# swoonge/SC-A-LOAM

Measured on AMD Instinct MI355X. Metric: scans/sec (feat-extract + scan-to-map ICP + SC loop search), KITTI HDL-64, higher is better.
Workload: dtype f32 points / f64 pose algebra

## Files before the change

sc-a-loam_amd/csrc/common.hpp:

```cpp
#pragma once
#include <hip/hip_runtime.h>
#include <hip/hip_ext.h>
#include <cstdio>
#include <cstdarg>
#include <cstring>
#include <string>
#include <vector>
#include <utility>
#include <mutex>
#include "../../include/scaloam_hip.h"
#include "batch.hpp"

namespace scal {
constexpr unsigned EV_DEVICE_ONLY = hipEventDisableTiming | hipEventDisableSystemFence;


void set_error(const char* fmt, ...);

#define SCAL_HIP(expr)                                                                         \
    do {                                                                                       \
        hipError_t _e = (expr);                                                                \
        if (_e != hipSuccess) {                                                                \
            ::scal::set_error("%s failed: %s (%s:%d)", #expr, hipGetErrorString(_e), __FILE__, __LINE__); \
            return SCAL_E_HIP;                                                                 \
        }                                                                                      \
    } while (0)

#define SCAL_TRY(expr)           \
    do {                         \
        int _rc = (expr);        \
        if (_rc != SCAL_OK) return _rc; \
    } while (0)

int select_device(int device);
enum class StreamLayout { Shared, PerStage };
enum { STAGE_FEATURES = 0, STAGE_SC = 1, STAGE_ODOM = 3, STAGE_MAP = 4, STAGE_MAP_PREFETCH = 2, STAGE_SC_FILTER = 5 };
int stage_lane(StreamLayout layout, int stage);
StreamLayout default_stream_layout();
int acquire_stream(int device, hipStream_t* out, int lane = 0);
void release_stream(int device, int lane = 0);
int odom_create(const scal_odom_config* cfg, StreamLayout layout, scal_odom_t** out);
int map_create(const scal_map_config* cfg, StreamLayout layout, scal_map_t** out);
int sc_create(const scal_sc_config* cfg, StreamLayout layout, scal_sc_t** out);
int icp_create_on_lane(const scal_icp_config* cfg, int lane, scal_icp_t** out);
int refine_create_on_lane(const scal_refine_config* cfg, int lane, scal_refine_t** out);
int posegraph_create_on_lane(const scal_posegraph_config* cfg, int lane, scal_posegraph_t** out);
struct ScFilterOut {
    const float *x, *y, *z, *w;
    const int* d_n;
    int cap;
};
int sc_insert_features_then(scal_sc_t* ctx, scal_features_t* feat, int (*after)(void* user, hipStream_t s, const ScFilterOut& ds), void* user);

struct LaneStream {
    hipStream_t s = nullptr;
    int device = 0, lane = 0;
    LaneStream() = default;
    LaneStream(LaneStream&& o) noexcept { *this = std::move(o); }
    LaneStream& operator=(LaneStream&& o) noexcept {
        release();
        std::swap(s, o.s);
        device = o.device, lane = o.lane;
        return *this;
    }
    ~LaneStream() { release(); }
    operator hipStream_t() const { return s; }
    int acquire(int dev, int ln) {
        release();
        device = dev, lane = ln;
        return acquire_stream(dev, &s, ln);
    }
    void release() {
        if (s) release_stream(device, lane);
        s = nullptr;
    }
};
struct Event {
    hipEvent_t e = nullptr;
    Event() = default;
    Event(Event&& o) noexcept { *this = std::move(o); }
    Event& operator=(Event&& o) noexcept {
        reset();
        std::swap(e, o.e);
        return *this;
    }
    ~Event() { reset(); }
    operator hipEvent_t() const { return e; }
    int create(unsigned flags) {
        reset();
        return ensure(flags);
    }
    int ensure(unsigned flags) {
        const hipError_t r = e ? hipSuccess : hipEventCreateWithFlags(&e, flags);
        if (r == hipSuccess) return SCAL_OK;
        set_error("hipEventCreateWithFlags failed: %s", hipGetErrorString(r));
        e = nullptr;
        return SCAL_E_HIP;
    }
    void reset() {
        if (e) (void)hipEventDestroy(e);
        e = nullptr;
    }
};

template <class T>
struct DevBuf {
    T* p = nullptr;
    size_t n = 0;
    DevBuf() = default;
    DevBuf(const DevBuf&) = delete;
    DevBuf& operator=(const DevBuf&) = delete;
    ~DevBuf() { release(); }
    void release() {
        if (p) (void)hipFree(p);
        p = nullptr;
        n = 0;
    }
    int alloc(size_t count) {
        release();
        if (count == 0) count = 1;
        hipError_t e = hipMalloc(reinterpret_cast<void**>(&p), count * sizeof(T));
        if (e != hipSuccess) {
            set_error("hipMalloc(%zu bytes) failed: %s", count * sizeof(T), hipGetErrorString(e));
            p = nullptr;
            return SCAL_E_HIP;
        }
        n = count;
        return SCAL_OK;
    }
    int zero(hipStream_t s) {
        hipError_t e = op_memset_async(p, 0, n * sizeof(T), s);
        if (e != hipSuccess) {
            set_error("hipMemsetAsync failed: %s", hipGetErrorString(e));
            return SCAL_E_HIP;
        }
        return SCAL_OK;
    }
};

template <class T>
struct PinBuf {
    T* p = nullptr;
    size_t n = 0;
    PinBuf() = default;
    PinBuf(const PinBuf&) = delete;
    PinBuf& operator=(const PinBuf&) = delete;
    ~PinBuf() {
        if (p) (void)hipHostFree(p);
    }
    int alloc(size_t count) {
        if (p) (void)hipHostFree(p);
        p = nullptr;
        if (count == 0) count = 1;
        hipError_t e = hipHostMalloc(reinterpret_cast<void**>(&p), count * sizeof(T), hipHostMallocDefault);
        if (e != hipSuccess) {
            set_error("hipHostMalloc(%zu bytes) failed: %s", count * sizeof(T), hipGetErrorString(e));
            p = nullptr;
            return SCAL_E_HIP;
        }
        n = count;
        return SCAL_OK;
    }
};

inline int div_up(int a, int b) { return (a + b - 1) / b; }

struct HostStage {
    PinBuf<unsigned char> pin;
    size_t used = 0;
    struct Item {
        void* dst;
        size_t off, bytes;
    };
    std::vector<Item> items;
    bool reserve(size_t total) {
        if (pin.p && pin.n >= total) return true;
        if (used) return false;
        if (pin.alloc(total) != SCAL_OK) {
            (void)hipGetLastError();
            return false;
        }
        return true;
    }
    hipError_t d2h(void* user, const void* dev, size_t bytes, hipStream_t s) {
        if (!bytes) return hipSuccess;
        const size_t need = (bytes + 255) & ~static_cast<size_t>(255);
        if (!pin.p || used + need > pin.n) return hipMemcpyAsync(user, dev, bytes, hipMemcpyDeviceToHost, s);
        const hipError_t e = hipMemcpyAsync(pin.p + used, dev, bytes, hipMemcpyDeviceToHost, s);
        items.push_back({user, used, bytes});
        used += need;
        return e;
    }
    hipError_t h2d(void* dev, const void* user, size_t bytes, hipStream_t s) {
        if (!bytes) return hipSuccess;
        const size_t need = (bytes + 255) & ~static_cast<size_t>(255);
        if (!pin.p || used + need > pin.n) return hipMemcpyAsync(dev, user, bytes, hipMemcpyHostToDevice, s);
        std::memcpy(pin.p + used, user, bytes);
        const hipError_t e = hipMemcpyAsync(dev, pin.p + used, bytes, hipMemcpyHostToDevice, s);
        used += need;
        return e;
    }
    void finish() {
        for (const Item& it : items) std::memcpy(it.dst, pin.p + it.off, it.bytes);
        items.clear();
        used = 0;
    }
};

bool prof_begin(const char* name, hipStream_t stream, hipEvent_t* start, hipEvent_t* stop);

#define SCAL_LAUNCH_PROF(name, kernel, grid, block, lds, stream, ...)                                   \
    do {                                                                                                \
        hipEvent_t pe0_ = nullptr, pe1_ = nullptr;                                                      \
        if (::scal::prof_begin(name, stream, &pe0_, &pe1_))                                                     \
            hipExtLaunchKernelGGL(kernel, grid, block, lds, stream, pe0_, pe1_, 0, __VA_ARGS__);        \
        else                                                                                            \
            hipLaunchKernelGGL(kernel, grid, block, lds, stream, __VA_ARGS__);                          \
    } while (0)

}
```

sc-a-loam_amd/csrc/odometry.hip:

```cpp
#include "common.hpp"
#include <deque>
#include "device_utils.hpp"
#include "voxel_dev.hpp"
#include "lm_host.hpp"
#include "features_dev.hpp"
#include <cmath>
#include <algorithm>

namespace scal {

struct OdomCounters {
    int n_corner_last, n_surf_last;
    int n_sharp, n_flat, n_less_sharp, n_less_flat;
    int n_slots, enable;
    int n_live[2], n_edge[2], n_plane[2];
};

__device__ __forceinline__ float sqdist(float ax, float ay, float az, float bx, float by, float bz) {
    return (ax - bx) * (ax - bx) + (ay - by) * (ay - by) + (az - bz) * (az - bz);
}

__device__ __forceinline__ unsigned long long make_key(float d, unsigned seq) {
    return (static_cast<unsigned long long>(__float_as_uint(d)) << 32) | seq;
}

constexpr int RING_TAB = 96;

__device__ __forceinline__ void transform_to_start(const double* x7, float ox, float oy, float oz, float* o) {
    double r[3];
    quat_rotate(x7, static_cast<double>(ox), static_cast<double>(oy), static_cast<double>(oz), r);
    o[0] = static_cast<float>(r[0] + 1.0 * x7[4]);
    o[1] = static_cast<float>(r[1] + 1.0 * x7[5]);
    o[2] = static_cast<float>(r[2] + 1.0 * x7[6]);
}

constexpr int OD_H = 8192;
constexpr int OD_LEVELS = 2;
__device__ constexpr float OD_INV_CELL[OD_LEVELS] = {1.0f, 0.2f};
__device__ constexpr float OD_EXACT_D2[OD_LEVELS] = {0.99f, 24.9f};
struct CellIndex {
    const int* start[OD_LEVELS];
    const float4* pts[OD_LEVELS];
};
__device__ __forceinline__ int od_cell(float v, int level) { return static_cast<int>(floorf(v * OD_INV_CELL[level])); }
__device__ __forceinline__ unsigned od_hash(int cx, int cy, int cz) {
    return (static_cast<unsigned>(cx) * 73856093u ^ static_cast<unsigned>(cy) * 19349663u ^ static_cast<unsigned>(cz) * 83492791u) & (OD_H - 1);
}
__device__ __forceinline__ unsigned od_bucket(float x, float y, float z, int level) { return od_hash(od_cell(x, level), od_cell(y, level), od_cell(z, level)); }
__device__ __forceinline__ unsigned long long od_cell_nn(const int* __restrict__ start, const float4* __restrict__ pts, int level, float sx, float sy, float sz,
                                                          int* s_beg, int* s_pre, unsigned long long* s_nn) {
    const int lane = lane_id(), wv = wave_id();
    if (wv == 0) {
        int b = 0, cnt = 0;
        if (lane < 27) {
            const unsigned h = od_hash(od_cell(sx, level) + lane % 3 - 1, od_cell(sy, level) + (lane / 3) % 3 - 1, od_cell(sz, level) + lane / 9 - 1);
            b = start[h];
            cnt = start[h + 1] - b;
        }
        int incl = cnt;
#pragma unroll
        for (int o = 1; o < 32; o <<= 1) {
            const int v = __shfl_up(incl, o, 64);
            if (lane >= o) incl += v;
        }
        if (lane < 27) s_beg[lane] = b, s_pre[lane + 1] = incl;
        if (lane == 0) s_pre[0] = 0;
    }
    __syncthreads();
    unsigned long long best = ~0ull;
    const int n_cand = s_pre[27];
    for (int m = threadIdx.x; m < n_cand; m += 256) {
        int j = 0;
#pragma unroll
        for (int o = 16; o >= 1; o >>= 1)
            if (j + o <= 26 && s_pre[j + o] <= m) j += o;
        const float4 p = pts[s_beg[j] + (m - s_pre[j])];
        const float dx = sx - p.x, dy = sy - p.y, dz = sz - p.z;
        float d = dx * dx;
        d += dy * dy;
        d += dz * dz;
        best = min(best, make_key(d, __float_as_uint(p.w)));
    }
    best = wave_min_u64(best);
    if (lane == 0) s_nn[wv] = best;
    __syncthreads();
    best = min(min(s_nn[0], s_nn[1]), min(s_nn[2], s_nn[3]));
    __syncthreads();
    return best;
}

__device__ __forceinline__ void k_odom_assoc_body(const CSoA4& sharp, const CSoA4& flat, const CSoA4& CL, const CSoA4& SL, const LMState* __restrict__ st, OdomCounters* C,
                                                    int outer, const FactorSoA& f, const CellIndex& ci_corner, const CellIndex& ci_surf,
                                                    const int* __restrict__ ring_tab) {
    if (!C->enable) return;
    const int ns = C->n_sharp, nf = C->n_flat;
    if (blockIdx.x == 0 && threadIdx.x == 0) C->n_slots = min(ns + nf, f.cap);
    __shared__ unsigned long long s_k2[4], s_k3[4];
    const int q = blockIdx.x;
    if (q >= ns + nf || q >= f.cap) return;
    const int lane = lane_id(), wv = wave_id();
    const bool is_edge = q < ns;
    const int j = is_edge ? q : q - ns;
    const CSoA4& Q = is_edge ? sharp : flat;
    const CSoA4& T = is_edge ? CL : SL;
    const int nT = is_edge ? C->n_corner_last : C->n_surf_last;
    double x7[7];
#pragma unroll
    for (int k = 0; k < 7; ++k) x7[k] = st->x[k];
    const float ox = Q.x[j], oy = Q.y[j], oz = Q.z[j];
    float sel[3];
    transform_to_start(x7, ox, oy, oz, sel);
    const float sx = sel[0], sy = sel[1], sz = sel[2];

    __shared__ int s_beg[27], s_pre[28];
    __shared__ unsigned long long s_nn[4];
    const CellIndex& ci = is_edge ? ci_corner : ci_surf;
    unsigned long long best = od_cell_nn(ci.start[0], ci.pts[0], 0, sx, sy, sz, s_beg, s_pre, s_nn);
    auto dist_of = [](unsigned long long k) { return __uint_as_float(static_cast<unsigned>(k >> 32)); };
    if (best == ~0ull || !(dist_of(best) < OD_EXACT_D2[0])) {
        best = od_cell_nn(ci.start[1], ci.pts[1], 1, sx, sy, sz, s_beg, s_pre, s_nn);
        if (best == ~0ull || !(dist_of(best) < OD_EXACT_D2[1])) {
            best = ~0ull;
            for (int t0 = threadIdx.x; t0 < nT; t0 += 1024) {
                float txx[4], tyy[4], tzz[4];
#pragma unroll
                for (int u = 0; u < 4; ++u) {
                    const int t = min(t0 + 256 * u, nT - 1);
                    txx[u] = T.x[t], tyy[u] = T.y[t], tzz[u] = T.z[t];
                }
#pragma unroll
                for (int u = 0; u < 4; ++u) {
                    const int t = min(t0 + 256 * u, nT - 1);
                    const float dx = sx - txx[u], dy = sy - tyy[u], dz = sz - tzz[u];
                    float d = dx * dx;
                    d += dy * dy;
                    d += dz * dz;
                    best = min(best, make_key(d, static_cast<unsigned>(t)));
                }
            }
            best = wave_min_u64(best);
            if (lane == 0) s_nn[wv] = best;
            __syncthreads();
            best = min(min(s_nn[0], s_nn[1]), min(s_nn[2], s_nn[3]));
        }
    }
    int valid = 0;
    int kind = is_edge ? 0 : 1;
    double pa[3] = {0, 0, 0}, pb[3] = {0, 0, 0};
    const float nnd = __uint_as_float(static_cast<unsigned>(best >> 32));
    if (best != ~0ull && static_cast<double>(nnd) < 25.0) {
        const int c = static_cast<int>(best & 0xffffffffu);
        const int id = static_cast<int>(T.w[c]);
        unsigned long long k2 = ~0ull, k3 = ~0ull;
        const int* first_idx = ring_tab + (is_edge ? 0 : 2 * RING_TAB);
        const int* last_idx = first_idx + RING_TAB;
        int fi = 0x7f7f7f7f, li = -1;
        for (int r = lane; r < RING_TAB; r += 64) {
            if (r >= id + 3) fi = min(fi, first_idx[r]);
            if (r <= id - 3) li = max(li, last_idx[r]);
        }
        const int hi = min(wave_min_i(fi), nT);
        const int lo = wave_max_i(li);
        for (int t0 = c + 1 + lane + 64 * wv; t0 < hi; t0 += 1024) {
            float tw[4], txx[4], tyy[4], tzz[4];
#pragma unroll
            for (int u = 0; u < 4; ++u) {
                const int t = t0 + 256 * u;
                if (t < hi) tw[u] = T.w[t], txx[u] = T.x[t], tyy[u] = T.y[t], tzz[u] = T.z[t];
            }
#pragma unroll
            for (int u = 0; u < 4; ++u) {
                const int t = t0 + 256 * u;
                if (t < hi) {
                    const int rj = static_cast<int>(tw[u]);
                    const float d = sqdist(txx[u], tyy[u], tzz[u], sx, sy, sz);
                    if (static_cast<double>(d) < 25.0) {
                        const unsigned seq = static_cast<unsigned>(t - c - 1);
                        if (is_edge) {
                            if (rj > id) k2 = min(k2, make_key(d, seq));
                        } else {
                            if (rj <= id) k2 = min(k2, make_key(d, seq));
                            else k3 = min(k3, make_key(d, seq));
                        }
                    }
                }
            }
        }
        for (int t0 = c - 1 - lane - 64 * wv; t0 > lo; t0 -= 1024) {
            float tw[4], txx[4], tyy[4], tzz[4];
#pragma unroll
            for (int u = 0; u < 4; ++u) {
                const int t = t0 - 256 * u;
                if (t > lo) tw[u] = T.w[t], txx[u] = T.x[t], tyy[u] = T.y[t], tzz[u] = T.z[t];
            }
#pragma unroll
            for (int u = 0; u < 4; ++u) {
                const int t = t0 - 256 * u;
                if (t > lo) {
                    const int rj = static_cast<int>(tw[u]);
                    const float d = sqdist(txx[u], tyy[u], tzz[u], sx, sy, sz);
                    if (static_cast<double>(d) < 25.0) {
                        const unsigned seq = 0x40000000u + static_cast<unsigned>(c - 1 - t);
                        if (is_edge) {
                            if (rj < id) k2 = min(k2, make_key(d, seq));
                        } else {
                            if (rj >= id) k2 = min(k2, make_key(d, seq));
                            else k3 = min(k3, make_key(d, seq));
                        }
                    }
                }
            }
        }
        k2 = wave_min_u64(k2);
        k3 = wave_min_u64(k3);
        if (lane == 0) s_k2[wv] = k2, s_k3[wv] = k3;
        __syncthreads();
        k2 = min(min(s_k2[0], s_k2[1]), min(s_k2[2], s_k2[3]));
        k3 = min(min(s_k3[0], s_k3[1]), min(s_k3[2], s_k3[3]));
        auto decode = [&](unsigned long long k) {
            const unsigned seq = static_cast<unsigned>(k & 0xffffffffu);
            return (seq & 0x40000000u) ? c - 1 - static_cast<int>(seq & 0x3fffffffu) : c + 1 + static_cast<int>(seq);
        };
        if (is_edge) {
            if (k2 != ~0ull) {
                const int i2 = decode(k2);
                valid = 1;
                pa[0] = T.x[c], pa[1] = T.y[c], pa[2] = T.z[c];
                pb[0] = T.x[i2], pb[1] = T.y[i2], pb[2] = T.z[i2];
            }
        } else if (k2 != ~0ull && k3 != ~0ull) {
            const int i2 = decode(k2), i3 = decode(k3);
            valid = 1;
            const double jx = T.x[c], jy = T.y[c], jz = T.z[c];
            const double lx = T.x[i2], ly = T.y[i2], lz = T.z[i2];
            const double mx = T.x[i3], my = T.y[i3], mz = T.z[i3];
            const double ax = jx - lx, ay = jy - ly, az = jz - lz, bx = jx - mx, by = jy - my, bz = jz - mz;
            double nx = ay * bz - az * by, ny = az * bx - ax * bz, nz = ax * by - ay * bx;
            const double z = nx * nx + ny * ny + nz * nz;
            if (z > 0) {
                const double s = sqrt(z);
                nx /= s, ny /= s, nz /= s;
            }
            pa[0] = jx, pa[1] = jy, pa[2] = jz;
            pb[0] = nx, pb[1] = ny, pb[2] = nz;
        }
    }
    if (lane == 0 && wv == 0) {
        f.valid[q] = valid;
        f.kind[q] = kind;
        f.cp[q] = ox, f.cp[f.cap + q] = oy, f.cp[2 * f.cap + q] = oz;
        f.pa[q] = pa[0], f.pa[f.cap + q] = pa[1], f.pa[2 * f.cap + q] = pa[2];
        f.pb[q] = pb[0], f.pb[f.cap + q] = pb[1], f.pb[2 * f.cap + q] = pb[2];
    }
}
SCAL_KERNEL(256, k_odom_assoc)

__device__ __forceinline__ void k_odom_init_pose_body(LMState* st, int* ring_tab) {
    if (threadIdx.x == 0) {
        st->x[0] = st->x[1] = st->x[2] = 0.0, st->x[3] = 1.0;
        st->x[4] = st->x[5] = st->x[6] = 0.0;
    }
    for (int t = threadIdx.x; t < 8 * RING_TAB; t += blockDim.x) ring_tab[t] = ((t / RING_TAB) & 1) ? -1 : 0x7f7f7f7f;
}
SCAL_KERNEL(1024, k_odom_init_pose)
struct HandoverArgs {
    CSoA4 in[2];
    const int* d_n[2];
    SoA4 out[2];
    int* d_n_out[2];
    int cap[2];
    int nb0;
    int* tab_write;
    int* tab_reset;
    const LMState* st;
    LMState* host_st;
    const LMSync* sync;
    int* cell_cnt[2][OD_LEVELS];
    int* cell_rank[2][OD_LEVELS];
};
__device__ __forceinline__ void k_odom_handover_body(const HandoverArgs& a) {
    int b = blockIdx.x;
    const int k = b < a.nb0 ? 0 : 1;
    if (k) b -= a.nb0;
    if (blockIdx.x == 0) {
        for (int t = threadIdx.x; t < 4 * RING_TAB; t += 256) a.tab_reset[t] = ((t / RING_TAB) & 1) ? -1 : 0x7f7f7f7f;
        const unsigned* src = reinterpret_cast<const unsigned*>(a.st);
        unsigned* dst = reinterpret_cast<unsigned*>(a.host_st);
        const bool abandoned = a.sync->abandoned != 0;
        constexpr int TERM_WORD = static_cast<int>(offsetof(LMState, termination) / 4);
        for (int t = threadIdx.x; t < static_cast<int>(sizeof(LMState) / 4); t += 256) dst[t] = (abandoned && t == TERM_WORD) ? 5u : src[t];
    }
    int* first_idx = a.tab_write + 2 * k * RING_TAB;
    int* last_idx = first_idx + RING_TAB;
    const CSoA4 in = a.in[k];
    const SoA4 out = a.out[k];
    const int n = min(*a.d_n[k], a.cap[k]);
    const int i = b * 256 + threadIdx.x;
    if (i == 0) *a.d_n_out[k] = n;
    if (b * 256 >= n) return;
    const int lane = lane_id();
    float x = 0, y = 0, z = 0;
    if (i < n) {
        const float w = in.w[i];
        x = in.x[i], y = in.y[i], z = in.z[i];
        out.x[i] = x, out.y[i] = y, out.z[i] = z, out.w[i] = w;
        const int r = min(max(static_cast<int>(w), 0), RING_TAB - 1);
        const int rp = __shfl_up(r, 1, 64);
        const int rn = __shfl_down(r, 1, 64);
        if (lane == 0 || rp != r) atomicMin(&first_idx[r], i);
        if (lane == 63 || rn != r || i == n - 1) atomicMax(&last_idx[r], i);
    }
#pragma unroll
    for (int l = 0; l < OD_LEVELS; ++l) {
        const unsigned h = i < n ? od_bucket(x, y, z, l) : 0xffffffffu;
        const unsigned hp = __shfl_up(h, 1, 64);
        const unsigned long long heads = __ballot(lane == 0 || hp != h);
        const int head = 63 - __clzll(heads & (~0ull >> (63 - lane)));
        const unsigned long long above = lane == 63 ? 0ull : heads & (~0ull << (lane + 1));
        const int next = above ? __ffsll(static_cast<long long>(above)) - 1 : 64;
        int base = 0;
        if (lane == head && i < n) {
            base = atomicAdd(&a.cell_cnt[k][l][h], next - head);
        }
        base = __shfl(base, head, 64);
        if (i < n) a.cell_rank[k][l][i] = base + (lane - head);
    }
}
SCAL_KERNEL(256, k_odom_handover)
constexpr int OD_START_STRIDE = OD_H + 4;
__device__ __forceinline__ void k_odom_cellscan_body(int* cnt_all, int* start_all) {
    constexpr int PER = OD_H / 1024;
    static_assert(PER % 4 == 0, "int4 loads");
    int* cnt = cnt_all + blockIdx.x * OD_H;
    int* start = start_all + blockIdx.x * OD_START_STRIDE;
    __shared__ int s_w[16];
    int v[PER];
    int4* c4 = reinterpret_cast<int4*>(cnt + threadIdx.x * PER);
    int sum = 0;
#pragma unroll
    for (int u = 0; u < PER / 4; ++u) {
        const int4 q = c4[u];
        v[4 * u] = q.x, v[4 * u + 1] = q.y, v[4 * u + 2] = q.z, v[4 * u + 3] = q.w;
        sum += q.x + q.y + q.z + q.w;
        c4[u] = make_int4(0, 0, 0, 0);
    }
    int incl = sum;
    const int lane = lane_id(), wv = wave_id();
#pragma unroll
    for (int o = 1; o < 64; o <<= 1) {
        const int t = __shfl_up(incl, o, 64);
        if (lane >= o) incl += t;
    }
    if (lane == 63) s_w[wv] = incl;
    __syncthreads();
    int base = incl - sum;
    for (int w = 0; w < wv; ++w) base += s_w[w];
    int4* s4 = reinterpret_cast<int4*>(start + threadIdx.x * PER);
#pragma unroll
    for (int u = 0; u < PER / 4; ++u) {
        int4 o;
        o.x = base, base += v[4 * u];
        o.y = base, base += v[4 * u + 1];
        o.z = base, base += v[4 * u + 2];
        o.w = base, base += v[4 * u + 3];
        s4[u] = o;
    }
    if (threadIdx.x == 1023) start[OD_H] = base;
}
SCAL_KERNEL(1024, k_odom_cellscan)
struct CellFillArgs {
    CSoA4 in[2];
    const int* d_n[2];
    const int* rank[2][OD_LEVELS];
    const int* start[2][OD_LEVELS];
    float4* pts[2][OD_LEVELS];
    int nb0;
};
__device__ __forceinline__ void k_odom_cellfill_body(const CellFillArgs& a) {
    int b = blockIdx.x;
    const int k = b < a.nb0 ? 0 : 1;
    if (k) b -= a.nb0;
    const int i = b * 256 + threadIdx.x;
    if (i >= *a.d_n[k]) return;
    const float x = a.in[k].x[i], y = a.in[k].y[i], z = a.in[k].z[i];
    const float4 rec = make_float4(x, y, z, __uint_as_float(static_cast<unsigned>(i)));
#pragma unroll
    for (int l = 0; l < OD_LEVELS; ++l) a.pts[k][l][a.start[k][l][od_bucket(x, y, z, l)] + a.rank[k][l][i]] = rec;
}
SCAL_KERNEL(256, k_odom_cellfill)
struct OdomGatherArgs {
    const float *sharp, *flat, *less;
    CSoA4 less_flat;
    const int *n_sharp, *n_flat, *n_less, *n_less_flat;
    SoA4 o_sharp, o_flat, o_less, o_less_flat;
    int slot_cap, feat_cap, cap, nbs, nbf;
};
__device__ __forceinline__ void k_odom_gather_body(const OdomGatherArgs& a, OdomCounters* C) {
    int b = blockIdx.x;
    const float* aos = nullptr;
    const int* d_n;
    int* d_n_out;
    SoA4 out;
    int cap;
    if (b < a.nbs) {
        aos = a.sharp, d_n = a.n_sharp, d_n_out = &C->n_sharp, out = a.o_sharp, cap = a.slot_cap;
        if (b == 0 && threadIdx.x == 0) {
            C->n_slots = 0, C->enable = 1;
            C->n_live[0] = C->n_live[1] = C->n_edge[0] = C->n_edge[1] = C->n_plane[0] = C->n_plane[1] = 0;
        }
    } else if (b < 2 * a.nbs) {
        b -= a.nbs, aos = a.flat, d_n = a.n_flat, d_n_out = &C->n_flat, out = a.o_flat, cap = a.slot_cap;
    } else if (b < 2 * a.nbs + a.nbf) {
        b -= 2 * a.nbs, aos = a.less, d_n = a.n_less, d_n_out = &C->n_less_sharp, out = a.o_less, cap = a.feat_cap;
    } else {
        b -= 2 * a.nbs + a.nbf, d_n = a.n_less_flat, d_n_out = &C->n_less_flat, out = a.o_less_flat, cap = a.cap;
    }
    const int n = min(*d_n, cap);
    const int i = b * 256 + threadIdx.x;
    if (i == 0) *d_n_out = n;
    if (i >= n) return;
    if (aos) {
        const float4 p = reinterpret_cast<const float4*>(aos)[i];
        out.x[i] = p.x, out.y[i] = p.y, out.z[i] = p.z, out.w[i] = p.w;
    } else {
        out.x[i] = a.less_flat.x[i], out.y[i] = a.less_flat.y[i], out.z[i] = a.less_flat.z[i], out.w[i] = a.less_flat.w[i];
    }
}
SCAL_KERNEL(256, k_odom_gather)

}

using namespace scal;

struct scal_odom {
    scal_odom_config cfg;
    LaneStream stream;
    int cap = 0, feat_cap = 0;
    bool systemInited = false;
    static constexpr int MAX_STEPS = 4;
    struct Pending {
        int slot;
        bool solve;
    };
    std::deque<Pending> pending;
    Event ev[MAX_STEPS];
    int next_slot = 0;
    double q_w_curr[4] = {0, 0, 0, 1}, t_w_curr[3] = {0, 0, 0};
    DevBuf<float> aos;
    SoAStore sharp, flat, less_sharp, less_flat;
    SoAStore corner_last, surf_last;
    LMStore lm;
    DevBuf<int> cell_cnt, cell_start, cell_rank;
    DevBuf<float4> cell_pts;
    int* cell_cnt_of(int k, int l) const { return cell_cnt.p + (k * OD_LEVELS + l) * OD_H; }
    int* cell_start_of(int k, int l) const { return cell_start.p + (k * OD_LEVELS + l) * OD_START_STRIDE; }
    int* cell_rank_of(int k, int l) const { return cell_rank.p + (size_t)l * (feat_cap + cap) + (k ? feat_cap : 0); }
    float4* cell_pts_of(int k, int l) const { return cell_pts.p + (size_t)l * (feat_cap + cap) + (k ? feat_cap : 0); }
    CellIndex cell_index(int k) const {
        CellIndex ci;
        for (int l = 0; l < OD_LEVELS; ++l) ci.start[l] = cell_start_of(k, l), ci.pts[l] = cell_pts_of(k, l);
        return ci;
    }
    DevBuf<int> ring_tab;
    int tab_cur = 0;
    DevBuf<OdomCounters> d_C;
    PinBuf<LMState> h_st;
    PinBuf<OdomCounters> h_up;
    HostStage hs;
    bool adapter_active = false, adapter_solve = false;
    BlockAdapter blocks;
    int outer_next = 0;
};

int scal::odom_create(const scal_odom_config* cfg, StreamLayout layout, scal_odom_t** out) {
    if (!cfg || !out || cfg->max_points <= 0) {
        set_error("scal_odom_create: bad argument");
        return SCAL_E_ARG;
    }
    *out = nullptr;
    SCAL_TRY(select_device(cfg->device));
    auto* c = new scal_odom();
    c->cfg = *cfg;
    c->cap = cfg->max_points;
    c->feat_cap = 120 * 64;
    int rc = SCAL_OK;
    auto A = [&](int r) { if (rc == SCAL_OK) rc = r; };
    A(c->lm.alloc(36 * 64));
    A(c->aos.alloc((size_t)c->cap * 4));
    A(c->sharp.alloc(c->lm.slot_cap)); A(c->flat.alloc(c->lm.slot_cap));
    A(c->less_sharp.alloc(c->feat_cap)); A(c->corner_last.alloc(c->feat_cap));
    A(c->less_flat.alloc(c->cap)); A(c->surf_last.alloc(c->cap));
    A(c->cell_cnt.alloc(2 * OD_LEVELS * OD_H)); A(c->cell_start.alloc(2 * OD_LEVELS * OD_START_STRIDE));
    A(c->cell_rank.alloc(OD_LEVELS * ((size_t)c->feat_cap + c->cap))); A(c->cell_pts.alloc(OD_LEVELS * ((size_t)c->feat_cap + c->cap)));
    A(c->ring_tab.alloc(8 * RING_TAB));
    A(c->blocks.alloc(c->lm.slot_cap));
    A(c->d_C.alloc(1)); A(c->h_st.alloc(scal_odom::MAX_STEPS)); A(c->h_up.alloc(1));
    if (rc == SCAL_OK) rc = lm_check_residency<LMNoHook, LMNoHook>(c->cfg.device);
    if (rc == SCAL_OK) rc = c->stream.acquire(c->cfg.device, stage_lane(layout, STAGE_ODOM));
    for (int k = 0; k < scal_odom::MAX_STEPS && rc == SCAL_OK; ++k) rc = c->ev[k].create(hipEventDisableTiming);
    if (rc == SCAL_OK) {
        rc = c->lm.init(c->stream);
        if (rc == SCAL_OK && op_memset_async(c->d_C.p, 0, sizeof(OdomCounters), c->stream) != hipSuccess) rc = SCAL_E_HIP;
        if (rc == SCAL_OK) rc = c->cell_cnt.zero(c->stream);
        if (rc == SCAL_OK) rc = c->cell_start.zero(c->stream);
        SCAL_LAUNCH("k_odom_init_pose", k_odom_init_pose, dim3(1), dim3(256), 0, c->stream, c->lm.d_st.p, c->ring_tab.p);
        if (rc == SCAL_OK && op_stream_synchronize(c->stream) != hipSuccess) rc = SCAL_E_HIP;
    }
    if (rc != SCAL_OK) {
        if (rc == SCAL_E_HIP) set_error("scal_odom_create: HIP resource creation failed");
        delete c;
        return rc;
    }
    *out = c;
    return SCAL_OK;
}

extern "C" int scal_odom_create(const scal_odom_config* cfg, scal_odom_t** out) { return odom_create(cfg, default_stream_layout(), out); }

extern "C" void scal_odom_destroy(scal_odom_t* c) {
    if (!c) return;
    (void)hipSetDevice(c->cfg.device);
    if (c->stream) (void)op_stream_synchronize(c->stream);
    delete c;
}

namespace {

int launch_handover(scal_odom* c, int slot, hipEvent_t ev);
int odom_enqueue(scal_odom* c) {
    hipStream_t s = c->stream;
    OdomCounters* C = c->d_C.p;
    LMState* st = c->lm.d_st.p;
    FactorSoA F = c->lm.factors();
    const bool solve = c->systemInited;
    c->systemInited = true;
    const int slot = c->next_slot;
    c->next_slot = (c->next_slot + 1) % scal_odom::MAX_STEPS;
    if (solve) {
        for (int outer = 0; outer < 2; ++outer) {
            {
                SCAL_LAUNCH("k_odom_assoc", k_odom_assoc, dim3(std::max(1, c->lm.slot_cap)), dim3(256), 0, s, c->sharp.cv(), c->flat.cv(),
                                   c->corner_last.cv(), c->surf_last.cv(), st, C, outer, F, c->cell_index(0), c->cell_index(1), c->ring_tab.p + c->tab_cur * 4 * RING_TAB);
            }
            {
                                launch_lm_solve(s, F, &C->n_slots, st, &C->enable, c->lm.partials.p, c->lm.lm_sync.p, outer, nullptr, LMNoHook(), LMNoHook(), "k_lm_solve_odom");
            }
        }
    }
    SCAL_TRY(launch_handover(c, slot, c->ev[slot]));
    c->pending.push_back({slot, solve});
    return SCAL_OK;
}

int launch_handover(scal_odom* c, int slot, hipEvent_t ev) {
    hipStream_t s = c->stream;
    OdomCounters* C = c->d_C.p;
    LMState* st = c->lm.d_st.p;
    {
        HandoverArgs h;
        h.in[0] = c->less_sharp.cv(), h.in[1] = c->less_flat.cv();
        h.d_n[0] = &C->n_less_sharp, h.d_n[1] = &C->n_less_flat;
        h.out[0] = c->corner_last.v(), h.out[1] = c->surf_last.v();
        h.d_n_out[0] = &C->n_corner_last, h.d_n_out[1] = &C->n_surf_last;
        h.cap[0] = c->feat_cap, h.cap[1] = c->cap;
        h.nb0 = std::max(1, div_up(c->feat_cap, 256));
        h.tab_write = c->ring_tab.p + (c->tab_cur ^ 1) * 4 * RING_TAB;
        h.tab_reset = c->ring_tab.p + c->tab_cur * 4 * RING_TAB;
        h.st = st, h.host_st = c->h_st.p + slot, h.sync = c->lm.lm_sync.p;
        for (int k = 0; k < 2; ++k)
            for (int l = 0; l < OD_LEVELS; ++l) h.cell_cnt[k][l] = c->cell_cnt_of(k, l), h.cell_rank[k][l] = c->cell_rank_of(k, l);
        const dim3 grid(h.nb0 + std::max(1, div_up(c->cap, 256)));
        SCAL_LAUNCH("k_odom_handover", k_odom_handover, grid, dim3(256), 0, s, h);
        c->tab_cur ^= 1;
        if (ev) SCAL_HIP(op_event_record(ev, s));
        SCAL_LAUNCH("k_odom_cellscan", k_odom_cellscan, dim3(2 * OD_LEVELS), dim3(1024), 0, s, c->cell_cnt.p, c->cell_start.p);
        CellFillArgs f;
        f.in[0] = c->corner_last.cv(), f.in[1] = c->surf_last.cv();
        f.d_n[0] = &C->n_corner_last, f.d_n[1] = &C->n_surf_last;
        for (int k = 0; k < 2; ++k)
            for (int l = 0; l < OD_LEVELS; ++l) f.rank[k][l] = c->cell_rank_of(k, l), f.start[k][l] = c->cell_start_of(k, l), f.pts[k][l] = c->cell_pts_of(k, l);
        f.nb0 = h.nb0;
        SCAL_LAUNCH("k_odom_cellfill", k_odom_cellfill, grid, dim3(256), 0, s, f);
    }
    SCAL_HIP(hipGetLastError());
    return SCAL_OK;
}

int odom_collect(scal_odom* c, double* q_lc, double* t_lc, double* q_w, double* t_w, scal_odom_stats* stats) {
    if (c->pending.empty()) {
        set_error("scal_odom_collect: no step enqueued");
        return SCAL_E_STATE;
    }
    const int slot = c->pending.front().slot;
    const bool solve = c->pending.front().solve;
    c->pending.pop_front();
    SCAL_HIP(op_event_synchronize(c->ev[slot]));
    const LMState& L = c->h_st.p[slot];
    if (L.termination == 5) {
        (void)c->lm.clear_exchange(c->stream);
        set_error("LM solve abandoned: grid barrier timed out");
        return SCAL_E_HIP;
    }
    const double* x = L.x;
    if (solve) {
        double r[3];
        q_rot(c->q_w_curr, x + 4, r);
        for (int i = 0; i < 3; ++i) c->t_w_curr[i] = c->t_w_curr[i] + r[i];
        double qn[4];
        q_mul(c->q_w_curr, x, qn);
        for (int i = 0; i < 4; ++i) c->q_w_curr[i] = qn[i];
    }
    for (int i = 0; i < 4; ++i) q_lc[i] = x[i], q_w[i] = c->q_w_curr[i];
    for (int i = 0; i < 3; ++i) t_lc[i] = x[4 + i], t_w[i] = c->t_w_curr[i];
    if (stats) {
        std::memset(stats, 0, sizeof *stats);
        if (solve) {
            for (int o = 0; o < 2; ++o) {
                stats->n_edge[o] = L.log_n_edge[o], stats->n_plane[o] = L.log_n_plane[o];
                stats->lm_iters[o] = L.log_iters[o], stats->lm_success[o] = L.log_success[o];
                stats->cost_init[o] = L.log_cost_init[o], stats->cost_final[o] = L.log_cost_final[o];
            }
        }
    }
    return SCAL_OK;
}

}

static int odom_upload(scal_odom* c, const float* sharp, int n_sharp, const float* less_sharp, int n_less_sharp, const float* flat, int n_flat,
                       const float* less_flat, int n_less_flat) {
    hipStream_t s = c->stream;
    SCAL_HIP(op_stream_synchronize(s));
    c->hs.finish();
    (void)c->hs.reserve(((size_t)2 * c->lm.slot_cap + c->feat_cap + c->cap) * 16 + 4096);
    OdomCounters& H = *c->h_up.p;
    OdomCounters fresh;
    std::memset(&fresh, 0, sizeof fresh);
    fresh.n_sharp = n_sharp, fresh.n_flat = n_flat, fresh.n_less_sharp = n_less_sharp, fresh.n_less_flat = n_less_flat, fresh.enable = 1;
    H = fresh;
    const size_t off = offsetof(OdomCounters, n_sharp);
    SCAL_HIP(op_memcpy_async(reinterpret_cast<char*>(c->d_C.p) + off, reinterpret_cast<char*>(&H) + off, sizeof(OdomCounters) - off,
                            hipMemcpyHostToDevice, s));
    auto up = [&](const float* src, int n, SoAStore& dst) -> int {
        if (n > 0) {
            SCAL_HIP(c->hs.h2d(c->aos.p, src, sizeof(float) * 4 * n, s));
            launch_deinterleave(s, c->aos.p, n, dst.v());
        }
        return SCAL_OK;
    };
    SCAL_TRY(up(sharp, n_sharp, c->sharp));
    SCAL_TRY(up(flat, n_flat, c->flat));
    SCAL_TRY(up(less_sharp, n_less_sharp, c->less_sharp));
    SCAL_TRY(up(less_flat, n_less_flat, c->less_flat));
    return SCAL_OK;
}

extern "C" int scal_odom_step(scal_odom_t* c, const float* sharp, int n_sharp, const float* less_sharp, int n_less_sharp, const float* flat,
                              int n_flat, const float* less_flat, int n_less_flat, double* q_lc, double* t_lc, double* q_w, double* t_w,
                              scal_odom_stats* stats) {
    if (!c || !q_lc || !t_lc || !q_w || !t_w || n_sharp < 0 || n_less_sharp < 0 || n_flat < 0 || n_less_flat < 0 || (n_sharp && !sharp) ||
        (n_less_sharp && !less_sharp) || (n_flat && !flat) || (n_less_flat && !less_flat)) {
        set_error("scal_odom_step: bad argument");
        return SCAL_E_ARG;
    }
    if (n_sharp + n_flat > c->lm.slot_cap || n_sharp > c->lm.slot_cap || n_flat > c->lm.slot_cap || n_less_sharp > c->feat_cap || n_less_flat > c->cap) {
        set_error("scal_odom_step: cloud larger than the context capacity (sharp+flat <= %d, lessSharp <= %d, lessFlat <= %d)", c->lm.slot_cap,
                  c->feat_cap, c->cap);
        return SCAL_E_TOO_MANY;
    }
    SCAL_HIP(hipSetDevice(c->cfg.device));
    if (!c->pending.empty()) {
        set_error("scal_odom_step: a queued step has not been collected");
        return SCAL_E_STATE;
    }
    SCAL_TRY(odom_upload(c, sharp, n_sharp, less_sharp, n_less_sharp, flat, n_flat, less_flat, n_less_flat));
    SCAL_TRY(odom_enqueue(c));
    return odom_collect(c, q_lc, t_lc, q_w, t_w, stats);
}

extern "C" int scal_odom_enqueue_features(scal_odom_t* c, scal_features_t* feat) {
    if (!c || !feat) {
        set_error("scal_odom_enqueue_features: null argument");
        return SCAL_E_ARG;
    }
    if (static_cast<int>(c->pending.size()) >= scal_odom::MAX_STEPS) {
        set_error("scal_odom_enqueue_features: %d steps are queued and not collected", scal_odom::MAX_STEPS);
        return SCAL_E_STATE;
    }
    FeatDeviceView v = features_view(feat);
    if (v.device != c->cfg.device) {
        set_error("features context lives on device %d, odometry context on %d", v.device, c->cfg.device);
        return SCAL_E_ARG;
    }
    SCAL_HIP(hipSetDevice(c->cfg.device));
    hipStream_t s = c->stream;
    OdomGatherArgs a;
    a.sharp = v.sharp_xyzi, a.flat = v.flat_xyzi, a.less = v.less_xyzi;
    a.less_flat = CSoA4{v.lfx, v.lfy, v.lfz, v.lfi};
    a.n_sharp = &v.P->n_sharp, a.n_flat = &v.P->n_flat, a.n_less = &v.P->n_less_sharp, a.n_less_flat = &v.P->n_less_flat;
    a.o_sharp = c->sharp.v(), a.o_flat = c->flat.v(), a.o_less = c->less_sharp.v(), a.o_less_flat = c->less_flat.v();
    a.slot_cap = c->lm.slot_cap, a.feat_cap = c->feat_cap, a.cap = std::min(c->cap, v.cap);
    a.nbs = std::max(1, div_up(c->lm.slot_cap, 256)), a.nbf = std::max(1, div_up(c->feat_cap, 256));
    SCAL_TRY(features_wait_done(feat, s));
    SCAL_LAUNCH("k_odom_gather", k_odom_gather, dim3(2 * a.nbs + a.nbf + std::max(1, div_up(a.cap, 256))), dim3(256), 0, s, a, c->d_C.p);
    SCAL_TRY(features_note_reader(feat, s));
    return odom_enqueue(c);
}

extern "C" int scal_odom_collect(scal_odom_t* c, double* q_lc, double* t_lc, double* q_w, double* t_w, scal_odom_stats* stats) {
    if (!c || !q_lc || !t_lc || !q_w || !t_w) {
        set_error("scal_odom_collect: null argument");
        return SCAL_E_ARG;
    }
    SCAL_HIP(hipSetDevice(c->cfg.device));
    return odom_collect(c, q_lc, t_lc, q_w, t_w, stats);
}

extern "C" int scal_odom_step_features(scal_odom_t* c, scal_features_t* feat, double* q_lc, double* t_lc, double* q_w, double* t_w,
                                       scal_odom_stats* stats) {
    if (!c || !feat || !q_lc || !t_lc || !q_w || !t_w) {
        set_error("scal_odom_step_features: null argument");
        return SCAL_E_ARG;
    }
    SCAL_TRY(scal_odom_enqueue_features(c, feat));
    return odom_collect(c, q_lc, t_lc, q_w, t_w, stats);
}

extern "C" int scal_odom_adapter_begin(scal_odom_t* c, const float* sharp, int n_sharp, const float* less_sharp, int n_less_sharp, const float* flat,
                                       int n_flat, const float* less_flat, int n_less_flat, double* q_last_curr, double* t_last_curr, int* need_solve) {
    if (!c || !q_last_curr || !t_last_curr || !need_solve || n_sharp < 0 || n_less_sharp < 0 || n_flat < 0 || n_less_flat < 0 || (n_sharp && !sharp) ||
        (n_less_sharp && !less_sharp) || (n_flat && !flat) || (n_less_flat && !less_flat)) {
        set_error("scal_odom_adapter_begin: bad argument");
        return SCAL_E_ARG;
    }
    if (n_sharp + n_flat > c->lm.slot_cap || n_less_sharp > c->feat_cap || n_less_flat > c->cap) {
        set_error("scal_odom_adapter_begin: cloud larger than the context capacity");
        return SCAL_E_TOO_MANY;
    }
    if (!c->pending.empty() || c->adapter_active) {
        set_error("scal_odom_adapter_begin: a step is still open");
        return SCAL_E_STATE;
    }
    SCAL_HIP(hipSetDevice(c->cfg.device));
    hipStream_t s = c->stream;
    SCAL_HIP(op_stream_synchronize(s));
    SCAL_TRY(odom_upload(c, sharp, n_sharp, less_sharp, n_less_sharp, flat, n_flat, less_flat, n_less_flat));
    SCAL_HIP(op_memcpy_async(c->h_st.p, c->lm.d_st.p, sizeof(LMState), hipMemcpyDeviceToHost, s));
    SCAL_HIP(op_stream_synchronize(s));
    for (int i = 0; i < 4; ++i) q_last_curr[i] = c->h_st.p->x[i];
    for (int i = 0; i < 3; ++i) t_last_curr[i] = c->h_st.p->x[4 + i];
    c->adapter_solve = c->systemInited;
    c->systemInited = true;
    *need_solve = c->adapter_solve ? 1 : 0;
    c->adapter_active = true;
    c->outer_next = 0;
    return SCAL_OK;
}

extern "C" int scal_odom_associate(scal_odom_t* c, const double* q_last_curr, const double* t_last_curr, int* n_blocks, int* n_residuals) {
    if (!c || !q_last_curr || !t_last_curr || !n_blocks || !n_residuals) {
        set_error("scal_odom_associate: null argument");
        return SCAL_E_ARG;
    }
    if (!c->adapter_active || !c->adapter_solve) {
        set_error("scal_odom_associate: no open step that needs a solve");
        return SCAL_E_STATE;
    }
    SCAL_HIP(hipSetDevice(c->cfg.device));
    hipStream_t s = c->stream;
    OdomCounters* C = c->d_C.p;
    LMState* st = c->lm.d_st.p;
    FactorSoA F = c->lm.factors();
    SCAL_TRY(c->blocks.set_pose(c->stream, c->lm.d_st.p->x, q_last_curr, t_last_curr));
    SCAL_LAUNCH("k_odom_assoc", k_odom_assoc, dim3(std::max(1, c->lm.slot_cap)), dim3(256), 0, s, c->sharp.cv(), c->flat.cv(), c->corner_last.cv(),
                     c->surf_last.cv(), st, C, std::min(c->outer_next, 1), F, c->cell_index(0), c->cell_index(1), c->ring_tab.p + c->tab_cur * 4 * RING_TAB);
    c->outer_next++;
    SCAL_TRY(c->blocks.compact(s, F, &C->n_slots));
    SCAL_HIP(op_stream_synchronize(s));
    *n_blocks = c->blocks.n_blocks(), *n_residuals = c->blocks.n_residuals();
    return SCAL_OK;
}

extern "C" int scal_odom_get_blocks(scal_odom_t* c, scal_block* out, int cap) {
    if (!c || (!out && cap > 0) || cap < 0) {
        set_error("scal_odom_get_blocks: bad argument");
        return SCAL_E_ARG;
    }
    if (!c->adapter_active) {
        set_error("scal_odom_get_blocks: no scal_odom_adapter_begin");
        return SCAL_E_STATE;
    }
    SCAL_HIP(hipSetDevice(c->cfg.device));
    return c->blocks.get_blocks(c->stream, c->lm.factors(), out, cap);
}

extern "C" int scal_odom_eval_blocks(scal_odom_t* c, const double* x7, int want_jac, double* residuals, double* jacobians) {
    if (!c || !x7 || !residuals || (want_jac && !jacobians)) {
        set_error("scal_odom_eval_blocks: bad argument");
        return SCAL_E_ARG;
    }
    if (!c->adapter_active) {
        set_error("scal_odom_eval_blocks: no scal_odom_adapter_begin");
        return SCAL_E_STATE;
    }
    SCAL_HIP(hipSetDevice(c->cfg.device));
    return c->blocks.eval_blocks(c->stream, c->lm.factors(), x7, want_jac, residuals, jacobians);
}

extern "C" int scal_odom_adapter_finish(scal_odom_t* c, const double* q_last_curr, const double* t_last_curr, double* q_w_curr, double* t_w_curr) {
    if (!c || !q_last_curr || !t_last_curr || !q_w_curr || !t_w_curr) {
        set_error("scal_odom_adapter_finish: null argument");
        return SCAL_E_ARG;
    }
    if (!c->adapter_active) {
        set_error("scal_odom_adapter_finish: no scal_odom_adapter_begin");
        return SCAL_E_STATE;
    }
    SCAL_HIP(hipSetDevice(c->cfg.device));
    c->adapter_active = false;
    SCAL_TRY(c->blocks.set_pose(c->stream, c->lm.d_st.p->x, q_last_curr, t_last_curr));
    const int slot = c->next_slot;
    c->next_slot = (c->next_slot + 1) % scal_odom::MAX_STEPS;
    SCAL_TRY(launch_handover(c, slot, c->ev[slot]));
    c->pending.push_back({slot, c->adapter_solve});
    double q_lc[4], t_lc[3];
    return odom_collect(c, q_lc, t_lc, q_w_curr, t_w_curr, nullptr);
}

extern "C" void* scal_odom_stream(scal_odom_t* c) { return c ? static_cast<void*>(c->stream) : nullptr; }
```

sc-a-loam_amd/csrc/pipeline.cpp:

```cpp
#include "common.hpp"
#include "keyframes.hpp"
#include <algorithm>
#include <cmath>
#include <condition_variable>
#include <deque>
#include <chrono>
#include <cstdlib>
#include <string>
#include <thread>

namespace scal {
void print_forced_flushes();
}
using namespace scal;

namespace {
constexpr int REC_N = 64;
constexpr int MAX_UNPOPPED = 32;
constexpr int MAX_LOOPS_UNPOPPED = 64;
int env_int(const char* name, int dflt, int lo, int hi) {
    const char* e = std::getenv(name);
    if (!e) return dflt;
    const int v = std::atoi(e);
    return v < lo ? lo : (v > hi ? hi : v);
}
const int B_AHEAD = env_int("SCALOAM_PIPE_B_AHEAD", 2, 1, 3);
const int PF_AHEAD = env_int("SCALOAM_PIPE_PF_AHEAD", 3, 1, 3);

const bool TIMING = env_int("SCALOAM_PIPE_TIMING", 0, 0, 1) != 0;
struct HostTimer {
    const char* name[12] = {};
    double total[12] = {};
    long calls[12] = {};
    template <class F>
    int run(int slot, const char* nm, F&& f) {
        if (!TIMING) return f();
        const auto t0 = std::chrono::steady_clock::now();
        const int rc = f();
        name[slot] = nm;
        total[slot] += std::chrono::duration<double, std::micro>(std::chrono::steady_clock::now() - t0).count();
        calls[slot]++;
        return rc;
    }
    void print(const char* thread) const {
        for (int i = 0; i < 12; ++i)
            if (calls[i]) std::fprintf(stderr, "[scal_pipeline] %-6s %-28s %8.1f us/call x %ld\n", thread, name[i], total[i] / calls[i], calls[i]);
    }
};

constexpr int SMAX = scal::BATCH_MAX;
struct Rec {
    const float* d_xyz[SMAX] = {};
    const void* h_xyz[SMAX] = {};
    int n[SMAX] = {};
    int stride = 0;
    bool host = false;
    scal_pipeline_result res[SMAX] = {};
};
}

struct scal_pipeline {
    scal_pipeline_config cfg{};
    int ring = 6, depth = 2;
    int S = 1;
    std::vector<scal_features_t*> regs[SMAX];
    scal_odom_t* od[SMAX] = {};
    scal_map_t* mp[SMAX] = {};
    scal_sc_t* sc[SMAX] = {};
    double* d_desc = nullptr;
    bool own_desc = false;
    Rec rec[REC_N];
    std::mutex mu;
    std::condition_variable cv;
    long long pushed = 0, a_run = 0, a_done = 0, pf_done = 0, b_enq = 0, b_coll = 0, c_enq = 0, c_coll = 0, d_ins = 0, d_coll = 0, popped = 0;
    int pop_waiting = 0;
    bool drain_req = false, drained = true;
    bool stop = false;
    int err = SCAL_OK;
    std::string errmsg;
    std::thread t_front, t_side, t_odom, t_pose, t_loop;
    HostTimer tm_front, tm_side, tm_odom, tm_pose, tm_loop;
    KeyframeStore* kf = nullptr;
    scal_keyframe_gate_state gate{};
    double fitness_thres = 0.3;
    std::deque<KfLoopJob> jobs;
    std::deque<scal_pipeline_loop> loops;
    bool verifying = false;
    long long verifying_seq = 0;
    long long loops_owed = 0;
    std::thread t_verify;
    struct AcceptedLoop {
        int curr_kf, loop_kf;
        double q[4], t[3];
    };
    std::vector<AcceptedLoop> accepted;
    int verifying_kf = -1;
    int kf_passed_end = 0;
    scal_posegraph_t* pg = nullptr;

    bool sc_on() const { return cfg.sc_mode != SCAL_PIPE_SC_OFF; }
    bool side_sc() const { return cfg.sc_mode == SCAL_PIPE_SC_EVERY_SCAN || cfg.sc_mode == SCAL_PIPE_SC_DESCRIPTOR; }
    bool kf_mode() const { return cfg.sc_mode == SCAL_PIPE_SC_KEYFRAME; }
    bool verify_idle() const { return jobs.empty() && !verifying; }
    Rec& r(long long k) { return rec[k % REC_N]; }
    template <class F>
    int for_all(F&& f) {
        if (S == 1) return f(0);
        Recorder recs[SMAX];
        Recorder* ptr[SMAX];
        int rc = SCAL_OK;
        for (int q = 0; q < S && rc == SCAL_OK; ++q) {
            ptr[q] = &recs[q];
            g_recorder = &recs[q];
            rc = f(q);
            g_recorder = nullptr;
        }
        if (rc != SCAL_OK) {
            for (int q = 0; q < S; ++q) (void)recs[q].flush();
            return rc;
        }
        if (zip_and_launch(ptr, S) != hipSuccess) {
            set_error("scal_pipeline: a batched launch failed: %s", hipGetErrorString(hipGetLastError()));
            return SCAL_E_HIP;
        }
        return SCAL_OK;
    }
    template <class F>
    int for_each(F&& f) {
        for (int q = 0; q < S; ++q) SCAL_TRY(f(q));
        return SCAL_OK;
    }
    void fail(int rc) {
        if (err == SCAL_OK) {
            err = rc;
            errmsg = scal_last_error();
        }
        cv.notify_all();
    }
};

namespace {

void front_thread(scal_pipeline* p) {
    std::unique_lock<std::mutex> lk(p->mu);
    for (;;) {
        const long long k = p->a_done;
        p->cv.wait(lk, [&] {
            if (p->stop || p->err) return true;
            if (p->pushed <= k) return false;
            const long long old = k - p->ring;
            if (old >= 0 && (p->c_coll <= old || p->b_enq <= old || (p->sc_on() && p->d_ins <= old))) return false;
            return k - p->c_enq < PF_AHEAD;
        });
        if (p->stop || p->err) return;
        const Rec& rc = p->r(k);
        const int slot = static_cast<int>(k % p->ring);
        lk.unlock();
        int st = p->tm_front.run(0, "A: features_run", [&] {
            return p->for_all([&](int q) {
                scal_features_t* reg = p->regs[q][slot];
                return rc.host ? scal_features_enqueue_host(reg, rc.h_xyz[q], rc.n[q], rc.stride) : scal_features_run_device(reg, rc.d_xyz[q], rc.n[q], rc.stride);
            });
        });
        if (st == SCAL_OK) {
            lk.lock();
            p->a_run = k + 1;
            p->cv.notify_all();
            lk.unlock();
            st = p->tm_front.run(1, "C: prefetch, lane 0 half", [&] { return p->for_all([&](int q) { return scal_map_prefetch_begin(p->mp[q], p->regs[q][slot]); }); });
        }
        lk.lock();
        if (st != SCAL_OK) {
            p->fail(st);
            return;
        }
        p->a_done = k + 1;
        p->cv.notify_all();
    }
}

void side_thread(scal_pipeline* p) {
    std::unique_lock<std::mutex> lk(p->mu);
    const bool search = p->cfg.sc_mode == SCAL_PIPE_SC_EVERY_SCAN;
    for (;;) {
        const long long k = p->pf_done;
        p->cv.wait(lk, [&] {
            if (p->stop || p->err) return true;
            if (p->a_done <= k) return false;
            return !(p->side_sc() && k - p->d_coll >= 3);
        });
        if (p->stop || p->err) return;
        const int slot = static_cast<int>(k % p->ring);
        lk.unlock();
        double* dd = p->d_desc ? p->d_desc + static_cast<size_t>(slot) * 1200 : nullptr;
        int st = p->tm_side.run(1, "C: prefetch, side half + D: insert", [&]() -> int {
            if (!p->side_sc() && p->S == 1) return scal_map_prefetch_finish(p->mp[0], p->regs[0][slot]);
            Recorder recs[2 * SMAX];
            Recorder* ptr[2 * SMAX];
            int nr = 0, rc2 = SCAL_OK;
            rc2 = p->tm_side.run(3, "   record prefetch", [&] {
                int r3 = SCAL_OK;
                for (int q = 0; q < p->S && r3 == SCAL_OK; ++q) {
                    g_recorder = ptr[nr] = &recs[nr];
                    ++nr;
                    r3 = scal_map_prefetch_finish(p->mp[q], p->regs[q][slot]);
                    g_recorder = nullptr;
                }
                return r3;
            });
            if (rc2 == SCAL_OK && p->side_sc())
                rc2 = p->tm_side.run(4, "   record insert", [&] {
                    int r3 = SCAL_OK;
                    for (int q = 0; q < p->S && r3 == SCAL_OK; ++q) {
                        g_recorder = ptr[nr] = &recs[nr];
                        ++nr;
                        r3 = search ? scal_sc_insert_features(p->sc[q], p->regs[q][slot]) : scal_sc_make_features_enqueue(p->sc[q], p->regs[q][slot], dd);
                        g_recorder = nullptr;
                    }
                    return r3;
                });
            if (rc2 != SCAL_OK) {
                for (int i = 0; i < nr; ++i) (void)recs[i].flush();
                return rc2;
            }
            return p->tm_side.run(5, "   zip + launch", [&]() -> int {
                if (zip_marked_and_launch(ptr, nr) != hipSuccess) {
                    set_error("scal_pipeline: a batched launch failed: %s", hipGetErrorString(hipGetLastError()));
                    return SCAL_E_HIP;
                }
                return SCAL_OK;
            });
        });
        if (st == SCAL_OK && search) st = p->tm_side.run(2, "D: sc_detect_enqueue", [&] { return p->for_all([&](int q) { return scal_sc_detect_enqueue(p->sc[q]); }); });
        lk.lock();
        if (st != SCAL_OK) {
            p->fail(st);
            return;
        }
        p->r(k).res[0].d_descriptor = dd;
        p->pf_done = k + 1;
        if (p->side_sc()) p->d_ins = k + 1;
        p->cv.notify_all();
    }
}

void odom_thread(scal_pipeline* p) {
    std::unique_lock<std::mutex> lk(p->mu);
    for (;;) {
        enum { NONE, B_ENQ, B_COLL } what = NONE;
        p->cv.wait(lk, [&] {
            if (p->stop || p->err) return true;
            if (p->b_enq < p->a_run && p->b_enq - p->b_coll < B_AHEAD) { what = B_ENQ; return true; }
            if (p->b_coll < p->b_enq && p->b_coll - p->c_enq < 2) { what = B_COLL; return true; }
            return false;
        });
        if (p->stop || p->err) return;
        int st = SCAL_OK;
        if (what == B_ENQ) {
            const long long k = p->b_enq;
            const int slot = static_cast<int>(k % p->ring);
            lk.unlock();
            st = p->tm_odom.run(0, "B: odom_enqueue_features", [&] { return p->for_all([&](int q) { return scal_odom_enqueue_features(p->od[q], p->regs[q][slot]); }); });
            lk.lock();
            if (st == SCAL_OK) p->b_enq = k + 1;
        } else {
            const long long k = p->b_coll;
            scal_pipeline_result* R = p->r(k).res;
            lk.unlock();
            st = p->tm_odom.run(1, "B: odom_collect (wait)", [&] {
                return p->for_each([&](int q) {
                    double qlc[4], tlc[3];
                    return scal_odom_collect(p->od[q], qlc, tlc, R[q].q_odom, R[q].t_odom, &R[q].odom);
                });
            });
            lk.lock();
            if (st == SCAL_OK) p->b_coll = k + 1;
        }
        if (st != SCAL_OK) {
            p->fail(st);
            return;
        }
        p->cv.notify_all();
    }
}

void pose_thread(scal_pipeline* p) {
    std::unique_lock<std::mutex> lk(p->mu);
    for (;;) {
        enum { NONE, C_ENQ, C_COLL, FINISH } what = NONE;
        p->cv.wait(lk, [&] {
            if (p->stop || p->err) return true;
            const long long inflight = p->c_enq - p->c_coll;
            if (p->c_enq < p->b_coll && p->c_enq < p->pf_done && inflight <= p->depth) { what = C_ENQ; return true; }
            if (inflight > p->depth || (inflight > 0 && (p->pop_waiting || p->drain_req) && p->c_enq == p->pushed)) { what = C_COLL; return true; }
            if (p->drain_req && p->c_coll == p->pushed) { what = FINISH; return true; }
            return false;
        });
        if (p->stop || p->err) return;
        int st = SCAL_OK;
        if (what == C_ENQ) {
            const long long k = p->c_enq;
            const int slot = static_cast<int>(k % p->ring);
            scal_pipeline_result* R = p->r(k).res;
            lk.unlock();
            st = p->tm_pose.run(2, "C: map_enqueue_features", [&] {
                return p->for_all([&](int q) { return scal_map_enqueue_features(p->mp[q], p->regs[q][slot], R[q].q_odom, R[q].t_odom); });
            });
            lk.lock();
            if (st == SCAL_OK) p->c_enq = k + 1;
        } else if (what == C_COLL) {
            const long long k = p->c_coll;
            scal_pipeline_result* R = p->r(k).res;
            lk.unlock();
            st = p->tm_pose.run(3, "C: map_collect (wait)", [&] {
                return p->for_each([&](int q) { return scal_map_collect(p->mp[q], R[q].q_w_curr, R[q].t_w_curr, &R[q].map); });
            });
            lk.lock();
            if (st == SCAL_OK) p->c_coll = k + 1;
        } else if (what == FINISH) {
            lk.unlock();
            st = p->for_each([&](int q) { return scal_map_finish(p->mp[q]); });
            lk.lock();
            if (st == SCAL_OK) p->drain_req = false, p->drained = true;
        }
        if (st != SCAL_OK) {
            p->fail(st);
            return;
        }
        p->cv.notify_all();
    }
}

void loop_thread(scal_pipeline* p) {
    std::unique_lock<std::mutex> lk(p->mu);
    const bool search = p->cfg.sc_mode == SCAL_PIPE_SC_EVERY_SCAN;
    for (;;) {
        p->cv.wait(lk, [&] {
            if (p->stop || p->err) return true;
            const long long infl = p->d_ins - p->d_coll;
            return infl >= 2 || (infl > 0 && (p->pop_waiting || p->drain_req));
        });
        if (p->stop || p->err) return;
        const long long k = p->d_coll;
        scal_pipeline_result* R = p->r(k).res;
        lk.unlock();
        int st;
        if (search) {
            st = p->tm_loop.run(2, "D: sc_detect_collect (wait)", [&] {
                return p->for_each([&](int q) {
                    const int rc = scal_sc_detect_collect(p->sc[q], &R[q].loop);
                    R[q].have_loop = rc == SCAL_OK;
                    return rc;
                });
            });
        } else {
            st = scal_sc_wait_descriptor(p->sc[0]);
        }
        lk.lock();
        if (st != SCAL_OK) {
            p->fail(st);
            return;
        }
        p->d_coll = k + 1;
        p->cv.notify_all();
    }
}

void keyframe_thread(scal_pipeline* p) {
    std::unique_lock<std::mutex> lk(p->mu);
    for (;;) {
        const long long k = p->d_coll;
        p->cv.wait(lk, [&] { return p->stop || p->err || p->c_coll > k; });
        if (p->stop || p->err) return;
        scal_pipeline_result& R = p->r(k).res[0];
        const int slot = static_cast<int>(k % p->ring);
        lk.unlock();
        int is_kf = 0;
        bool detect = false;
        int st = scal_keyframe_gate(&p->gate, R.q_w_curr, R.t_w_curr, &is_kf);
        R.is_keyframe = is_kf, R.keyframe_id = -1, R.have_loop = 0;
        if (st == SCAL_OK && is_kf) {
            const int id = scal_sc_size(p->sc[0]);
            double p6[6];
            pose6_from(R.q_w_curr, R.t_w_curr, p6);
            st = p->tm_loop.run(0, "D: insert + append", [&] { return p->kf->insert(p->sc[0], p->regs[0][slot], id, p6); });
            if (st == SCAL_OK) {
                R.keyframe_id = id;
                detect = p->kf->own_count() >= 30;
                if (detect) st = p->tm_loop.run(1, "D: sc_detect_enqueue", [&] { return scal_sc_detect_enqueue(p->sc[0]); });
            }
        }
        lk.lock();
        if (st != SCAL_OK) {
            p->fail(st);
            return;
        }
        p->d_ins = k + 1;
        p->cv.notify_all();
        lk.unlock();
        if (detect) {
            st = p->tm_loop.run(2, "D: sc_detect_collect (wait)", [&] { return scal_sc_detect_collect(p->sc[0], &R.loop); });
            R.have_loop = st == SCAL_OK;
        }
        if (st == SCAL_OK && is_kf) st = p->kf->check();
        lk.lock();
        if (st != SCAL_OK) {
            p->fail(st);
            return;
        }
        if (detect && R.loop.loop_id >= 0) {
            p->jobs.push_back(KfLoopJob{k, R.keyframe_id, R.loop.loop_id, R.loop.yaw_rad, R.loop.min_dist});
            p->loops_owed++;
        }
        if (is_kf) p->kf_passed_end = R.keyframe_id + 1;
        p->d_coll = k + 1;
        p->cv.notify_all();
    }
}

void verify_thread(scal_pipeline* p) {
    std::unique_lock<std::mutex> lk(p->mu);
    for (;;) {
        p->cv.wait(lk, [&] { return p->stop || p->err || !p->jobs.empty(); });
        if (p->stop || p->err) return;
        const KfLoopJob job = p->jobs.front();
        p->jobs.pop_front();
        p->verifying = true, p->verifying_seq = job.seq, p->verifying_kf = job.curr_kf;
        lk.unlock();
        scal_pipeline_loop rec;
        const int st = p->kf->verify(job, p->fitness_thres, &rec);
        lk.lock();
        p->verifying = false;
        if (st != SCAL_OK) {
            p->fail(st);
            return;
        }
        p->loops.push_back(rec);
        if (rec.verified == 1) {
            scal_pipeline::AcceptedLoop a{rec.curr_kf, rec.loop_kf, {rec.q_rel[0], rec.q_rel[1], rec.q_rel[2], rec.q_rel[3]}, {rec.t_rel[0], rec.t_rel[1], rec.t_rel[2]}};
            p->accepted.push_back(a);
        }
        p->cv.notify_all();
    }
}

int report(scal_pipeline* p) {
    set_error("%s", p->errmsg.c_str());
    return p->err;
}

int push(scal_pipeline* p, const float* const* d_xyz, const void* const* h_xyz, const int* n, int stride, bool host) {
    std::unique_lock<std::mutex> lk(p->mu);
    if (p->err) return report(p);
    if (p->pushed - p->popped >= MAX_UNPOPPED) {
        set_error("scal_pipeline_push: %d results wait to be popped", MAX_UNPOPPED);
        return SCAL_E_STATE;
    }
    if (p->loops_owed >= MAX_LOOPS_UNPOPPED) {
        set_error("scal_pipeline_push: %d loop records wait to be popped (scal_pipeline_pop_loop)", MAX_LOOPS_UNPOPPED);
        return SCAL_E_STATE;
    }
    const long long k = p->pushed;
    Rec& rc = p->r(k);
    rc = Rec();
    for (int q = 0; q < p->S; ++q) {
        rc.d_xyz[q] = d_xyz ? d_xyz[q] : nullptr, rc.h_xyz[q] = h_xyz ? h_xyz[q] : nullptr, rc.n[q] = n[q];
        rc.res[q].seq = k;
    }
    rc.stride = stride, rc.host = host;
    p->pushed = k + 1;
    p->drained = false;
    p->cv.notify_all();
    p->cv.wait(lk, [&] { return p->err || (host ? p->a_done > k : p->a_done + p->ring > k); });
    if (p->err) return report(p);
    return SCAL_OK;
}

int pop(scal_pipeline* p, scal_pipeline_result* out) {
    std::unique_lock<std::mutex> lk(p->mu);
    if (p->popped >= p->pushed && !p->err) {
        set_error("scal_pipeline_pop: nothing pushed");
        return SCAL_E_STATE;
    }
    const long long k = p->popped;
    p->pop_waiting++;
    p->cv.notify_all();
    p->cv.wait(lk, [&] { return p->err || (p->c_coll > k && (!p->sc_on() || p->d_coll > k)); });
    p->pop_waiting--;
    if (p->err) return report(p);
    for (int q = 0; q < p->S; ++q) out[q] = p->r(k).res[q];
    p->popped = k + 1;
    p->cv.notify_all();
    return SCAL_OK;
}

int create(const scal_pipeline_config* cfg, int n_seqs, scal_pipeline_t** out) {
    if (!cfg || !out) {
        set_error("scal_pipeline_create: null argument");
        return SCAL_E_ARG;
    }
    *out = nullptr;
    const int ring = cfg->ring == 0 ? 6 : cfg->ring, depth = cfg->depth == 0 ? 2 : cfg->depth;
    if (ring < 4 || ring > 16 || depth < 1 || depth > 3 || cfg->sc_mode < 0 || cfg->sc_mode > 3) {
        set_error("scal_pipeline_create: ring must be 4..16, depth 1..3, sc_mode 0..3");
        return SCAL_E_ARG;
    }
    if (n_seqs < 1 || n_seqs > SMAX || (n_seqs > 1 && (cfg->sc_mode == SCAL_PIPE_SC_DESCRIPTOR || cfg->sc_mode == SCAL_PIPE_SC_KEYFRAME))) {
        set_error("scal_pipeline_create_multi: 1..%d sequences (sc_mode 2 and 3 only with one)", SMAX);
        return SCAL_E_ARG;
    }
    scal_keyframe_gate_state gate{};
    if (cfg->sc_mode == SCAL_PIPE_SC_KEYFRAME) {
        if (cfg->kf_max_points < 0 || !(cfg->loop_fitness_thres >= 0) || cfg->sc_max_keyframes <= 0 ||
            scal_keyframe_gate_init(&gate, cfg->keyframe_meter_gap == 0 ? 2.0 : cfg->keyframe_meter_gap,
                                    cfg->keyframe_deg_gap == 0 ? 10.0 : cfg->keyframe_deg_gap) != SCAL_OK) {
            set_error("scal_pipeline_create: sc_mode 3 needs keyframe gaps >= 0, kf_max_points >= 0, loop_fitness_thres >= 0, sc_max_keyframes > 0");
            return SCAL_E_ARG;
        }
    }
    if (cfg->pgo_map_max_points < 0 || (cfg->pgo_map_max_points > 0 && (cfg->sc_mode != SCAL_PIPE_SC_KEYFRAME || cfg->kf_max_points == 0))) {
        set_error("scal_pipeline_create: pgo_map_max_points must be >= 0, and > 0 only in sc_mode 3 with kf_max_points > 0");
        return SCAL_E_ARG;
    }
    SCAL_TRY(select_device(cfg->device));
    auto* p = new scal_pipeline();
    p->cfg = *cfg, p->ring = ring, p->depth = depth, p->S = n_seqs;
    p->gate = gate;
    p->fitness_thres = cfg->loop_fitness_thres == 0 ? 0.3 : cfg->loop_fitness_thres;
    int rc = SCAL_OK;
    if (p->kf_mode()) {
        p->kf = new KeyframeStore();
        rc = p->kf->init(cfg->device, cfg->kf_max_points, cfg->sc_max_keyframes, cfg->pgo_map_max_points);
    }
    scal_features_config fc{};
    fc.lidar_type = cfg->lidar_type, fc.n_scans = cfg->n_scans, fc.minimum_range = cfg->minimum_range, fc.max_points = cfg->max_points;
    fc.float_math = cfg->float_math, fc.check_finite = cfg->check_finite, fc.device = cfg->device;
    for (int q = 0; q < n_seqs && rc == SCAL_OK; ++q) {
        for (int i = 0; i < ring && rc == SCAL_OK; ++i) {
            scal_features_t* f = nullptr;
            rc = scal_features_create(&fc, &f);
            if (rc == SCAL_OK) p->regs[q].push_back(f);
        }
        if (rc == SCAL_OK) {
            scal_odom_config oc{};
            oc.max_points = cfg->max_points, oc.device = cfg->device;
            rc = odom_create(&oc, StreamLayout::PerStage, &p->od[q]);
        }
        if (rc == SCAL_OK) {
            scal_map_config mc{};
            mc.line_res = cfg->line_res, mc.plane_res = cfg->plane_res, mc.max_scan_points = cfg->max_points, mc.max_map_points = cfg->max_map_points;
            mc.device = cfg->device;
            rc = map_create(&mc, StreamLayout::PerStage, &p->mp[q]);
        }
        if (rc == SCAL_OK && p->sc_on()) {
            scal_sc_config sc{};
            sc.max_radius = cfg->sc_max_radius, sc.dist_thres = cfg->sc_dist_thres, sc.max_keyframes = cfg->sc_max_keyframes;
            sc.float_math = cfg->float_math, sc.device = cfg->device, sc.n_shards = 1, sc.shard = 0, sc.side_stream = env_int("SCALOAM_PIPE_SC_LANE", 1, 0, 5);
            rc = sc_create(&sc, StreamLayout::PerStage, &p->sc[q]);
            if (rc == SCAL_OK && cfg->sc_mode == SCAL_PIPE_SC_DESCRIPTOR) {
                if (cfg->d_desc_ring) {
                    p->d_desc = cfg->d_desc_ring;
                } else if (hipMalloc(reinterpret_cast<void**>(&p->d_desc), sizeof(double) * 1200 * ring) != hipSuccess) {
                    set_error("scal_pipeline_create: hipMalloc of the descriptor ring failed");
                    rc = SCAL_E_HIP;
                } else {
                    p->own_desc = true;
                }
            }
        }
    }
    if (rc != SCAL_OK) {
        const std::string keep = scal_last_error();
        scal_pipeline_destroy(p);
        set_error("%s", keep.c_str());
        return rc;
    }
    p->t_front = std::thread(front_thread, p);
    p->t_side = std::thread(side_thread, p);
    p->t_odom = std::thread(odom_thread, p);
    p->t_pose = std::thread(pose_thread, p);
    if (p->side_sc()) p->t_loop = std::thread(loop_thread, p);
    if (p->kf_mode()) p->t_loop = std::thread(keyframe_thread, p), p->t_verify = std::thread(verify_thread, p);
    *out = p;
    return SCAL_OK;
}

}

extern "C" int scal_pipeline_create(const scal_pipeline_config* cfg, scal_pipeline_t** out) { return create(cfg, 1, out); }
extern "C" int scal_pipeline_create_multi(const scal_pipeline_config* cfg, int n_seqs, scal_pipeline_t** out) { return create(cfg, n_seqs, out); }
extern "C" int scal_pipeline_seqs(scal_pipeline_t* p) { return p ? p->S : 0; }

extern "C" void scal_pipeline_destroy(scal_pipeline_t* p) {
    if (!p) return;
    {
        std::lock_guard<std::mutex> lk(p->mu);
        p->stop = true;
        p->cv.notify_all();
    }
    if (p->t_front.joinable()) p->t_front.join();
    if (p->t_side.joinable()) p->t_side.join();
    if (p->t_odom.joinable()) p->t_odom.join();
    if (p->t_pose.joinable()) p->t_pose.join();
    if (p->t_loop.joinable()) p->t_loop.join();
    if (p->t_verify.joinable()) p->t_verify.join();
    if (TIMING) {
        p->tm_front.print("front"), p->tm_side.print("side"), p->tm_odom.print("odom"), p->tm_pose.print("pose"), p->tm_loop.print("loop");
        std::fprintf(stderr, "[scal_pipeline] sequences %d, recorded lists flushed in the middle of an entry point: %ld\n", p->S, g_forced_flushes);
        print_forced_flushes();
    }
    (void)hipSetDevice(p->cfg.device);
    for (int q = 0; q < SMAX; ++q) {
        if (p->sc[q]) scal_sc_destroy(p->sc[q]);
        if (p->mp[q]) scal_map_destroy(p->mp[q]);
        if (p->od[q]) scal_odom_destroy(p->od[q]);
    }
    for (int q = 0; q < SMAX; ++q)
        for (auto* f : p->regs[q]) scal_features_destroy(f);
    if (p->pg) scal_posegraph_destroy(p->pg);
    delete p->kf;
    if (p->d_desc && p->own_desc) (void)hipFree(p->d_desc);
    delete p;
}

static int check_scan(scal_pipeline_t* p, const void* ptr, int n) {
    if ((!ptr && n > 0) || n < 0) {
        set_error("scal_pipeline_push: bad argument");
        return SCAL_E_ARG;
    }
    if (n > p->cfg.max_points) {
        set_error("scan has %d points, capacity is %d", n, p->cfg.max_points);
        return SCAL_E_TOO_MANY;
    }
    return SCAL_OK;
}

extern "C" int scal_pipeline_push_device(scal_pipeline_t* p, const float* d_xyz, int n, int stride_floats) {
    if (!p || stride_floats < 3 || p->S != 1) {
        set_error("scal_pipeline_push_device: bad argument (a pipeline of several sequences takes scal_pipeline_push_device_multi)");
        return SCAL_E_ARG;
    }
    SCAL_TRY(check_scan(p, d_xyz, n));
    return push(p, &d_xyz, nullptr, &n, stride_floats, false);
}

extern "C" int scal_pipeline_push_device_multi(scal_pipeline_t* p, const float* const* d_xyz, const int* n, int stride_floats) {
    if (!p || !d_xyz || !n || stride_floats < 3) {
        set_error("scal_pipeline_push_device_multi: bad argument");
        return SCAL_E_ARG;
    }
    for (int q = 0; q < p->S; ++q) SCAL_TRY(check_scan(p, d_xyz[q], n[q]));
    return push(p, d_xyz, nullptr, n, stride_floats, false);
}

extern "C" int scal_pipeline_push_host(scal_pipeline_t* p, const void* xyz, int n, int stride_bytes) {
    if (!p || stride_bytes < 12 || (stride_bytes % 4) != 0 || stride_bytes > 32 || p->S != 1) {
        set_error("scal_pipeline_push_host: bad argument (stride_bytes must be a multiple of 4 in [12, 32]; one sequence)");
        return SCAL_E_ARG;
    }
    SCAL_TRY(check_scan(p, xyz, n));
    return push(p, nullptr, &xyz, &n, stride_bytes, true);
}

extern "C" int scal_pipeline_pop(scal_pipeline_t* p, scal_pipeline_result* out) {
    if (!p || !out || p->S != 1) {
        set_error("scal_pipeline_pop: bad argument (a pipeline of several sequences takes scal_pipeline_pop_multi)");
        return SCAL_E_ARG;
    }
    return pop(p, out);
}

extern "C" int scal_pipeline_pop_multi(scal_pipeline_t* p, scal_pipeline_result* out) {
    if (!p || !out) {
        set_error("scal_pipeline_pop_multi: null argument");
        return SCAL_E_ARG;
    }
    return pop(p, out);
}

extern "C" int scal_pipeline_drain(scal_pipeline_t* p) {
    if (!p) return SCAL_E_ARG;
    std::unique_lock<std::mutex> lk(p->mu);
    if (p->err) return report(p);
    if (p->drained) return SCAL_OK;
    p->drain_req = true;
    p->pop_waiting++;
    p->cv.notify_all();
    p->cv.wait(lk, [&] { return p->err || (p->drained && (!p->sc_on() || p->d_coll == p->pushed) && p->verify_idle()); });
    p->pop_waiting--;
    if (p->err) return report(p);
    return SCAL_OK;
}

extern "C" int scal_pipeline_pop_loop(scal_pipeline_t* p, scal_pipeline_loop* out, int wait) {
    if (!p || !out) {
        set_error("scal_pipeline_pop_loop: null argument");
        return SCAL_E_ARG;
    }
    std::unique_lock<std::mutex> lk(p->mu);
    if (!p->kf_mode()) {
        set_error("scal_pipeline_pop_loop: only in sc_mode 3");
        return SCAL_E_STATE;
    }
    for (;;) {
        if (p->err) return report(p);
        if (!p->loops.empty()) {
            *out = p->loops.front();
            p->loops.pop_front();
            p->loops_owed--;
            return 1;
        }
        if (!wait || p->verify_idle()) return 0;
        p->cv.wait(lk);
    }
}

extern "C" int scal_pipeline_keyframe(scal_pipeline_t* p, int kf, double pose6[6], float* xyzi, int cap, int* n) {
    if (!p || !pose6 || !n || cap < 0 || (cap > 0 && !xyzi)) {
        set_error("scal_pipeline_keyframe: bad argument");
        return SCAL_E_ARG;
    }
    std::lock_guard<std::mutex> lk(p->mu);
    if (p->err) return report(p);
    if (!p->kf_mode() || !p->drained || p->d_coll != p->pushed || !p->verify_idle()) {
        set_error("scal_pipeline_keyframe: only in sc_mode 3, while the pipeline is drained");
        return SCAL_E_STATE;
    }
    return p->kf->read(kf, pose6, xyzi, cap, n);
}

static int update_poses_locked(scal_pipeline_t* p, const int* kf, const double* pose6, int n);

extern "C" int scal_pipeline_update_keyframe_poses(scal_pipeline_t* p, const int* kf, const double* pose6, int n) {
    if (!p || n < 0 || (n > 0 && (!kf || !pose6))) {
        set_error("scal_pipeline_update_keyframe_poses: bad argument");
        return SCAL_E_ARG;
    }
    std::lock_guard<std::mutex> lk(p->mu);
    if (p->err) return report(p);
    if (!p->kf_mode()) {
        set_error("scal_pipeline_update_keyframe_poses: only in sc_mode 3");
        return SCAL_E_STATE;
    }
    return update_poses_locked(p, kf, pose6, n);
}

static int update_poses_locked(scal_pipeline_t* p, const int* kf, const double* pose6, int n) {
    long long floor = p->d_coll;
    if (!p->jobs.empty()) floor = std::min(floor, p->jobs.front().seq);
    if (p->verifying) floor = std::min(floor, p->verifying_seq);
    return p->kf->update_poses(kf, pose6, n, p->pushed, floor);
}

static int pgo_map_state(scal_pipeline_t* p) {
    std::lock_guard<std::mutex> lk(p->mu);
    if (p->err) return report(p);
    if (!p->kf_mode() || p->cfg.pgo_map_max_points == 0) {
        set_error("scal_pipeline_pgo_map: only in sc_mode 3 with pgo_map_max_points > 0");
        return SCAL_E_STATE;
    }
    return SCAL_OK;
}

extern "C" int scal_pipeline_pgo_map(scal_pipeline_t* p, int kf_end, int skip, float leaf, float* out_xyzi, long long cap, long long* n_out) {
    if (!p || !n_out || cap < 0 || (cap > 0 && !out_xyzi)) {
        set_error("scal_pipeline_pgo_map: bad argument");
        return SCAL_E_ARG;
    }
    *n_out = 0;
    SCAL_TRY(pgo_map_state(p));
    if (!(leaf > 0.f) || !std::isfinite(leaf) || skip < 1 || kf_end < 0) {
        set_error("scal_pipeline_pgo_map: leaf must be finite and > 0, skip >= 1, kf_end >= 0");
        return SCAL_E_ARG;
    }
    return p->kf->pgo_map(kf_end, skip, leaf, out_xyzi, cap, n_out);
}

extern "C" const float* scal_pipeline_pgo_map_device(scal_pipeline_t* p, long long* n) {
    if (n) *n = 0;
    if (!p || !n || !p->kf_mode() || p->cfg.pgo_map_max_points == 0) return nullptr;
    return p->kf->pgo_map_device(n);
}

namespace {
void pose7_from6(const double* p6, double* p7) {
    const double cr = std::cos(p6[3] / 2), sr = std::sin(p6[3] / 2), cp = std::cos(p6[4] / 2), sp = std::sin(p6[4] / 2);
    const double cy = std::cos(p6[5] / 2), sy = std::sin(p6[5] / 2);
    p7[0] = sr * cp * cy - cr * sp * sy, p7[1] = cr * sp * cy + sr * cp * sy, p7[2] = cr * cp * sy - sr * sp * cy, p7[3] = cr * cp * cy + sr * sp * sy;
    p7[4] = p6[0], p7[5] = p6[1], p7[6] = p6[2];
}
void pose7_between(const double* a, const double* b, double* o) {
    const double x = -a[0], y = -a[1], z = -a[2], w = a[3];
    o[0] = w * b[0] + x * b[3] + y * b[2] - z * b[1];
    o[1] = w * b[1] - x * b[2] + y * b[3] + z * b[0];
    o[2] = w * b[2] + x * b[1] - y * b[0] + z * b[3];
    o[3] = w * b[3] - x * b[0] - y * b[1] - z * b[2];
    const double d[3] = {b[4] - a[4], b[5] - a[5], b[6] - a[6]};
    const double R[3][3] = {{1 - 2 * (y * y + z * z), 2 * (x * y - w * z), 2 * (x * z + w * y)},
                            {2 * (x * y + w * z), 1 - 2 * (x * x + z * z), 2 * (y * z - w * x)},
                            {2 * (x * z - w * y), 2 * (y * z + w * x), 1 - 2 * (x * x + y * y)}};
    for (int r = 0; r < 3; ++r) o[4 + r] = (R[r][0] * d[0] + R[r][1] * d[1]) + R[r][2] * d[2];
}
}

extern "C" int scal_pipeline_optimize_keyframes(scal_pipeline_t* p, int kf_end, int apply, int* kf_ids, double* pose6, int cap, scal_pipeline_pgo_result* res) {
    if (res) std::memset(res, 0, sizeof *res);
    if (!p || cap < 0 || (cap > 0 && (!kf_ids || !pose6))) {
        set_error("scal_pipeline_optimize_keyframes: bad argument");
        return SCAL_E_ARG;
    }
    {
        std::lock_guard<std::mutex> lk(p->mu);
        if (p->err) return report(p);
        if (!p->kf_mode()) {
            set_error("scal_pipeline_optimize_keyframes: only in sc_mode 3");
            return SCAL_E_STATE;
        }
    }
    if (kf_end < 0) {
        set_error("scal_pipeline_optimize_keyframes: kf_end must be >= 0");
        return SCAL_E_ARG;
    }
    std::vector<int> ids;
    std::vector<std::array<double, 6>> gated, current;
    SCAL_TRY(p->kf->pgo_snapshot(kf_end, &ids, &gated, &current));
    const int n = static_cast<int>(ids.size());
    if (res) res->n_nodes = n;
    if (cap < n) {
        set_error("scal_pipeline_optimize_keyframes: %d keyframes, room for %d", n, cap);
        return SCAL_E_CAPACITY;
    }
    if (n == 0) return SCAL_OK;
    std::vector<scal_pipeline::AcceptedLoop> loops;
    {
        std::unique_lock<std::mutex> lk(p->mu);
        const int need = ids.back() + 1;
        auto pending = [&] {
            if (p->verifying && p->verifying_kf < kf_end) return true;
            for (const KfLoopJob& j : p->jobs)
                if (j.curr_kf < kf_end) return true;
            return false;
        };
        p->cv.wait(lk, [&] { return p->err || p->stop || (p->kf_passed_end >= need && !pending()); });
        if (p->err) return report(p);
        if (p->stop) {
            set_error("scal_pipeline_optimize_keyframes: the pipeline is being destroyed");
            return SCAL_E_STATE;
        }
        for (const auto& a : p->accepted)
            if (a.curr_kf < kf_end) loops.push_back(a);
    }
    std::vector<double> x7(7 * static_cast<size_t>(n)), g7(7 * static_cast<size_t>(n));
    scal_posegraph_stats st{};
    {
        std::lock_guard<std::mutex> map_lk(p->kf->map_mu);
        SCAL_TRY(p->kf->pgo_snapshot(kf_end, &ids, &gated, &current));
        for (int k = 0; k < n; ++k) pose7_from6(gated[static_cast<size_t>(k)].data(), &g7[7 * static_cast<size_t>(k)]), pose7_from6(current[static_cast<size_t>(k)].data(), &x7[7 * static_cast<size_t>(k)]);
        if (!p->pg) {
            scal_posegraph_config pc{};
            pc.device = p->cfg.device, pc.max_nodes = p->cfg.sc_max_keyframes, pc.max_edges = 2 * p->cfg.sc_max_keyframes;
            SCAL_TRY(posegraph_create_on_lane(&pc, 2, &p->pg));
        }
        const double var_prior[6] = {1e-12, 1e-12, 1e-12, 1e-12, 1e-12, 1e-12};
        const double var_odom[6] = {1e-6, 1e-6, 1e-6, 1e-4, 1e-4, 1e-4};
        const double var_loop[6] = {0.5, 0.5, 0.5, 0.5, 0.5, 0.5};
        const size_t m = static_cast<size_t>(n - 1) + loops.size();
        std::vector<int> ei(m), ej(m);
        std::vector<double> ez(7 * m), ev(6 * m), ek(m);
        for (int k = 1; k < n; ++k) {
            const size_t e = static_cast<size_t>(k - 1);
            ei[e] = k - 1, ej[e] = k, ek[e] = 0.0;
            pose7_between(&g7[7 * e], &g7[7 * (e + 1)], &ez[7 * e]);
            std::memcpy(&ev[6 * e], var_odom, sizeof var_odom);
        }
        size_t e = static_cast<size_t>(n - 1);
        for (const auto& a : loops) {
            const auto node = [&](int db) { return static_cast<int>(std::lower_bound(ids.begin(), ids.end(), db) - ids.begin()); };
            ei[e] = node(a.loop_kf), ej[e] = node(a.curr_kf), ek[e] = 1.0;
            std::memcpy(&ez[7 * e], a.q, sizeof a.q), std::memcpy(&ez[7 * e + 4], a.t, sizeof a.t);
            std::memcpy(&ev[6 * e], var_loop, sizeof var_loop);
            ++e;
        }
        SCAL_TRY(scal_posegraph_set_nodes(p->pg, x7.data(), n));
        SCAL_TRY(scal_posegraph_clear_edges(p->pg));
        SCAL_TRY(scal_posegraph_set_prior(p->pg, 0, g7.data(), var_prior));
        SCAL_TRY(scal_posegraph_add_between(p->pg, static_cast<int>(m), ei.data(), ej.data(), ez.data(), ev.data(), ek.data()));
        SCAL_TRY(scal_posegraph_optimize(p->pg, nullptr, &st));
        SCAL_TRY(scal_posegraph_get_nodes(p->pg, x7.data(), n));
    }
    for (int k = 0; k < n; ++k) {
        kf_ids[k] = ids[static_cast<size_t>(k)];
        pose6_from(&x7[7 * static_cast<size_t>(k)], &x7[7 * static_cast<size_t>(k) + 4], pose6 + 6 * static_cast<size_t>(k));
    }
    if (res) res->n_odom_edges = n - 1, res->n_loop_edges = static_cast<int>(loops.size()), res->solver = st;
    if (apply) {
        std::lock_guard<std::mutex> lk(p->mu);
        if (p->err) return report(p);
        SCAL_TRY(update_poses_locked(p, kf_ids, pose6, n));
        if (res) res->applied = 1;
    }
    return SCAL_OK;
}

extern "C" int scal_pipeline_in_flight(scal_pipeline_t* p) {
    if (!p) return 0;
    std::lock_guard<std::mutex> lk(p->mu);
    return static_cast<int>(p->pushed - p->popped);
}

static bool seq_ok(scal_pipeline_t* p, int q) { return p && q >= 0 && q < p->S; }
extern "C" scal_sc_t* scal_pipeline_sc(scal_pipeline_t* p) { return p ? p->sc[0] : nullptr; }
extern "C" scal_map_t* scal_pipeline_map(scal_pipeline_t* p) { return p ? p->mp[0] : nullptr; }
extern "C" scal_odom_t* scal_pipeline_odom(scal_pipeline_t* p) { return p ? p->od[0] : nullptr; }
extern "C" scal_features_t* scal_pipeline_features(scal_pipeline_t* p, int i) {
    return (p && i >= 0 && i < static_cast<int>(p->regs[0].size())) ? p->regs[0][i] : nullptr;
}
extern "C" scal_sc_t* scal_pipeline_sc_of(scal_pipeline_t* p, int seq) { return seq_ok(p, seq) ? p->sc[seq] : nullptr; }
extern "C" scal_map_t* scal_pipeline_map_of(scal_pipeline_t* p, int seq) { return seq_ok(p, seq) ? p->mp[seq] : nullptr; }
```

Baseline: 4360.

## Prepare odometry target sets in front thread with ring of sets and paired batched launches

```diff
diff --git a/sc-a-loam_amd/csrc/common.hpp b/sc-a-loam_amd/csrc/common.hpp
--- a/sc-a-loam_amd/csrc/common.hpp
+++ b/sc-a-loam_amd/csrc/common.hpp
@@ -42,6 +42,9 @@
 int odom_create(const scal_odom_config* cfg, StreamLayout layout, scal_odom_t** out);
 int map_create(const scal_map_config* cfg, StreamLayout layout, scal_map_t** out);
 int sc_create(const scal_sc_config* cfg, StreamLayout layout, scal_sc_t** out);
+constexpr int ODOM_TARGET_SETS = 4;
+int odom_prepare_features(scal_odom_t* ctx, scal_features_t* feat, bool own_stream, long long scan);
+int odom_enqueue_prepared(scal_odom_t* ctx);
 int icp_create_on_lane(const scal_icp_config* cfg, int lane, scal_icp_t** out);
 int refine_create_on_lane(const scal_refine_config* cfg, int lane, scal_refine_t** out);
 int posegraph_create_on_lane(const scal_posegraph_config* cfg, int lane, scal_posegraph_t** out);
diff --git a/sc-a-loam_amd/csrc/odometry.hip b/sc-a-loam_amd/csrc/odometry.hip
--- a/sc-a-loam_amd/csrc/odometry.hip
+++ b/sc-a-loam_amd/csrc/odometry.hip
@@ -1,4 +1,5 @@
 #include "common.hpp"
+#include <atomic>
 #include <deque>
 #include "device_utils.hpp"
 #include "voxel_dev.hpp"
@@ -10,10 +11,10 @@
 namespace scal {
 
 struct OdomCounters {
-    int n_corner_last, n_surf_last;
+    int n_slots, enable;
+};
+struct SetCounts {
     int n_sharp, n_flat, n_less_sharp, n_less_flat;
-    int n_slots, enable;
-    int n_live[2], n_edge[2], n_plane[2];
 };
 
 __device__ __forceinline__ float sqdist(float ax, float ay, float az, float bx, float by, float bz) {
@@ -90,10 +91,10 @@
 }
 
 __device__ __forceinline__ void k_odom_assoc_body(const CSoA4& sharp, const CSoA4& flat, const CSoA4& CL, const CSoA4& SL, const LMState* __restrict__ st, OdomCounters* C,
-                                                    int outer, const FactorSoA& f, const CellIndex& ci_corner, const CellIndex& ci_surf,
+                                                    const SetCounts* __restrict__ nq, const SetCounts* __restrict__ nt, int outer, const FactorSoA& f, const CellIndex& ci_corner, const CellIndex& ci_surf,
                                                     const int* __restrict__ ring_tab) {
     if (!C->enable) return;
-    const int ns = C->n_sharp, nf = C->n_flat;
+    const int ns = nq->n_sharp, nf = nq->n_flat;
     if (blockIdx.x == 0 && threadIdx.x == 0) C->n_slots = min(ns + nf, f.cap);
     __shared__ unsigned long long s_k2[4], s_k3[4];
     const int q = blockIdx.x;
@@ -103,7 +104,7 @@
     const int j = is_edge ? q : q - ns;
     const CSoA4& Q = is_edge ? sharp : flat;
     const CSoA4& T = is_edge ? CL : SL;
-    const int nT = is_edge ? C->n_corner_last : C->n_surf_last;
+    const int nT = is_edge ? nt->n_less_sharp : nt->n_less_flat;
     double x7[7];
 #pragma unroll
     for (int k = 0; k < 7; ++k) x7[k] = st->x[k];
@@ -255,55 +256,64 @@
 }
 SCAL_KERNEL(256, k_odom_assoc)
 
-__device__ __forceinline__ void k_odom_init_pose_body(LMState* st, int* ring_tab) {
+constexpr int OD_SETS = ODOM_TARGET_SETS;
+__device__ __forceinline__ void k_odom_init_pose_body(LMState* st, int* ring_tab, OdomCounters* C) {
     if (threadIdx.x == 0) {
         st->x[0] = st->x[1] = st->x[2] = 0.0, st->x[3] = 1.0;
         st->x[4] = st->x[5] = st->x[6] = 0.0;
-    }
-    for (int t = threadIdx.x; t < 8 * RING_TAB; t += blockDim.x) ring_tab[t] = ((t / RING_TAB) & 1) ? -1 : 0x7f7f7f7f;
+        C->n_slots = 0, C->enable = 1;
+    }
+    for (int t = threadIdx.x; t < OD_SETS * 4 * RING_TAB; t += blockDim.x) ring_tab[t] = ((t / RING_TAB) & 1) ? -1 : 0x7f7f7f7f;
 }
 SCAL_KERNEL(1024, k_odom_init_pose)
-struct HandoverArgs {
-    CSoA4 in[2];
-    const int* d_n[2];
-    SoA4 out[2];
-    int* d_n_out[2];
-    int cap[2];
-    int nb0;
-    int* tab_write;
-    int* tab_reset;
-    const LMState* st;
-    LMState* host_st;
-    const LMSync* sync;
+struct OdomPrepArgs {
+    const float *sharp, *flat, *less;
+    const float* less_flat_aos;
+    CSoA4 less_flat;
+    const int *n_sharp, *n_flat, *n_less, *n_less_flat;
+    int n_host[4];
+    SoA4 o_sharp, o_flat, o_less, o_less_flat;
+    SetCounts* cnt;
+    int slot_cap, feat_cap, cap, nbs, nbf;
+    int* tab;
     int* cell_cnt[2][OD_LEVELS];
     int* cell_rank[2][OD_LEVELS];
 };
-__device__ __forceinline__ void k_odom_handover_body(const HandoverArgs& a) {
+__device__ __forceinline__ void k_odom_prepare_body(const OdomPrepArgs& a) {
     int b = blockIdx.x;
-    const int k = b < a.nb0 ? 0 : 1;
-    if (k) b -= a.nb0;
-    if (blockIdx.x == 0) {
-        for (int t = threadIdx.x; t < 4 * RING_TAB; t += 256) a.tab_reset[t] = ((t / RING_TAB) & 1) ? -1 : 0x7f7f7f7f;
-        const unsigned* src = reinterpret_cast<const unsigned*>(a.st);
-        unsigned* dst = reinterpret_cast<unsigned*>(a.host_st);
-        const bool abandoned = a.sync->abandoned != 0;
-        constexpr int TERM_WORD = static_cast<int>(offsetof(LMState, termination) / 4);
-        for (int t = threadIdx.x; t < static_cast<int>(sizeof(LMState) / 4); t += 256) dst[t] = (abandoned && t == TERM_WORD) ? 5u : src[t];
-    }
-    int* first_idx = a.tab_write + 2 * k * RING_TAB;
+    const float* aos = nullptr;
+    const int* d_n;
+    int n_host, cap, k = -1;
+    int* d_n_out;
+    SoA4 out;
+    if (b < a.nbs) {
+        aos = a.sharp, d_n = a.n_sharp, n_host = a.n_host[0], d_n_out = &a.cnt->n_sharp, out = a.o_sharp, cap = a.slot_cap;
+    } else if (b < 2 * a.nbs) {
+        b -= a.nbs, aos = a.flat, d_n = a.n_flat, n_host = a.n_host[1], d_n_out = &a.cnt->n_flat, out = a.o_flat, cap = a.slot_cap;
+    } else if (b < 2 * a.nbs + a.nbf) {
+        b -= 2 * a.nbs, aos = a.less, d_n = a.n_less, n_host = a.n_host[2], d_n_out = &a.cnt->n_less_sharp, out = a.o_less, cap = a.feat_cap, k = 0;
+    } else {
+        b -= 2 * a.nbs + a.nbf, aos = a.less_flat_aos, d_n = a.n_less_flat, n_host = a.n_host[3], d_n_out = &a.cnt->n_less_flat, out = a.o_less_flat, cap = a.cap, k = 1;
+    }
+    const int n = min(d_n ? *d_n : n_host, cap);
+    const int i = b * 256 + threadIdx.x;
+    if (i == 0) *d_n_out = n;
+    if (b * 256 >= n) return;
+    float x = 0, y = 0, z = 0, w = 0;
+    if (i < n) {
+        if (aos) {
+            const float4 p = reinterpret_cast<const float4*>(aos)[i];
+            x = p.x, y = p.y, z = p.z, w = p.w;
+        } else {
+            x = a.less_flat.x[i], y = a.less_flat.y[i], z = a.less_flat.z[i], w = a.less_flat.w[i];
+        }
+        out.x[i] = x, out.y[i] = y, out.z[i] = z, out.w[i] = w;
+    }
+    if (k < 0) return;
+    int* first_idx = a.tab + 2 * k * RING_TAB;
     int* last_idx = first_idx + RING_TAB;
-    const CSoA4 in = a.in[k];
-    const SoA4 out = a.out[k];
-    const int n = min(*a.d_n[k], a.cap[k]);
-    const int i = b * 256 + threadIdx.x;
-    if (i == 0) *a.d_n_out[k] = n;
-    if (b * 256 >= n) return;
     const int lane = lane_id();
-    float x = 0, y = 0, z = 0;
     if (i < n) {
-        const float w = in.w[i];
-        x = in.x[i], y = in.y[i], z = in.z[i];
-        out.x[i] = x, out.y[i] = y, out.z[i] = z, out.w[i] = w;
         const int r = min(max(static_cast<int>(w), 0), RING_TAB - 1);
         const int rp = __shfl_up(r, 1, 64);
         const int rn = __shfl_down(r, 1, 64);
@@ -326,7 +336,17 @@
         if (i < n) a.cell_rank[k][l][i] = base + (lane - head);
     }
 }
-SCAL_KERNEL(256, k_odom_handover)
+SCAL_KERNEL(256, k_odom_prepare)
+__device__ __forceinline__ void k_odom_publish_body(int* tab_reset, const LMState* st, LMState* host_st, const LMSync* sync) {
+    if (tab_reset)
+        for (int t = threadIdx.x; t < 4 * RING_TAB; t += 256) tab_reset[t] = ((t / RING_TAB) & 1) ? -1 : 0x7f7f7f7f;
+    const unsigned* src = reinterpret_cast<const unsigned*>(st);
+    unsigned* dst = reinterpret_cast<unsigned*>(host_st);
+    const bool abandoned = sync->abandoned != 0;
+    constexpr int TERM_WORD = static_cast<int>(offsetof(LMState, termination) / 4);
+    for (int t = threadIdx.x; t < static_cast<int>(sizeof(LMState) / 4); t += 256) dst[t] = (abandoned && t == TERM_WORD) ? 5u : src[t];
+}
+SCAL_KERNEL(256, k_odom_publish)
 constexpr int OD_START_STRIDE = OD_H + 4;
 __device__ __forceinline__ void k_odom_cellscan_body(int* cnt_all, int* start_all) {
     constexpr int PER = OD_H / 1024;
@@ -388,45 +408,6 @@
     for (int l = 0; l < OD_LEVELS; ++l) a.pts[k][l][a.start[k][l][od_bucket(x, y, z, l)] + a.rank[k][l][i]] = rec;
 }
 SCAL_KERNEL(256, k_odom_cellfill)
-struct OdomGatherArgs {
-    const float *sharp, *flat, *less;
-    CSoA4 less_flat;
-    const int *n_sharp, *n_flat, *n_less, *n_less_flat;
-    SoA4 o_sharp, o_flat, o_less, o_less_flat;
-    int slot_cap, feat_cap, cap, nbs, nbf;
-};
-__device__ __forceinline__ void k_odom_gather_body(const OdomGatherArgs& a, OdomCounters* C) {
-    int b = blockIdx.x;
-    const float* aos = nullptr;
-    const int* d_n;
-    int* d_n_out;
-    SoA4 out;
-    int cap;
-    if (b < a.nbs) {
-        aos = a.sharp, d_n = a.n_sharp, d_n_out = &C->n_sharp, out = a.o_sharp, cap = a.slot_cap;
-        if (b == 0 && threadIdx.x == 0) {
-            C->n_slots = 0, C->enable = 1;
-            C->n_live[0] = C->n_live[1] = C->n_edge[0] = C->n_edge[1] = C->n_plane[0] = C->n_plane[1] = 0;
-        }
-    } else if (b < 2 * a.nbs) {
-        b -= a.nbs, aos = a.flat, d_n = a.n_flat, d_n_out = &C->n_flat, out = a.o_flat, cap = a.slot_cap;
-    } else if (b < 2 * a.nbs + a.nbf) {
-        b -= 2 * a.nbs, aos = a.less, d_n = a.n_less, d_n_out = &C->n_less_sharp, out = a.o_less, cap = a.feat_cap;
-    } else {
-        b -= 2 * a.nbs + a.nbf, d_n = a.n_less_flat, d_n_out = &C->n_less_flat, out = a.o_less_flat, cap = a.cap;
-    }
-    const int n = min(*d_n, cap);
-    const int i = b * 256 + threadIdx.x;
-    if (i == 0) *d_n_out = n;
-    if (i >= n) return;
-    if (aos) {
-        const float4 p = reinterpret_cast<const float4*>(aos)[i];
-        out.x[i] = p.x, out.y[i] = p.y, out.z[i] = p.z, out.w[i] = p.w;
-    } else {
-        out.x[i] = a.less_flat.x[i], out.y[i] = a.less_flat.y[i], out.z[i] = a.less_flat.z[i], out.w[i] = a.less_flat.w[i];
-    }
-}
-SCAL_KERNEL(256, k_odom_gather)
 
 }
 
@@ -444,28 +425,48 @@
     };
     std::deque<Pending> pending;
     Event ev[MAX_STEPS];
-    int next_slot = 0;
     double q_w_curr[4] = {0, 0, 0, 1}, t_w_curr[3] = {0, 0, 0};
     DevBuf<float> aos;
-    SoAStore sharp, flat, less_sharp, less_flat;
-    SoAStore corner_last, surf_last;
+    static constexpr int R = OD_SETS;
+    static_assert(MAX_STEPS <= R, "a pose event must not be recorded again before the prepare that waits for it is queued");
+    struct TargetSet {
+        SoAStore sharp, flat, less_sharp, less_flat;
+        DevBuf<int> cell_cnt, cell_start, cell_rank;
+        DevBuf<float4> cell_pts;
+        int feat_cap = 0, cap = 0;
+        Event ready;
+        hipStream_t prep_stream = nullptr;
+        int* cell_cnt_of(int k, int l) const { return cell_cnt.p + (k * OD_LEVELS + l) * OD_H; }
+        int* cell_start_of(int k, int l) const { return cell_start.p + (k * OD_LEVELS + l) * OD_START_STRIDE; }
+        int* cell_rank_of(int k, int l) const { return cell_rank.p + (size_t)l * (feat_cap + cap) + (k ? feat_cap : 0); }
+        float4* cell_pts_of(int k, int l) const { return cell_pts.p + (size_t)l * (feat_cap + cap) + (k ? feat_cap : 0); }
+        CellIndex cell_index(int k) const {
+            CellIndex ci;
+            for (int l = 0; l < OD_LEVELS; ++l) ci.start[l] = cell_start_of(k, l), ci.pts[l] = cell_pts_of(k, l);
+            return ci;
+        }
+        int alloc(int slot_cap, int fc, int c) {
+            feat_cap = fc, cap = c;
+            SCAL_TRY(sharp.alloc(slot_cap));
+            SCAL_TRY(flat.alloc(slot_cap));
+            SCAL_TRY(less_sharp.alloc(fc));
+            SCAL_TRY(less_flat.alloc(c));
+            SCAL_TRY(cell_cnt.alloc(2 * OD_LEVELS * OD_H));
+            SCAL_TRY(cell_start.alloc(2 * OD_LEVELS * OD_START_STRIDE));
+            SCAL_TRY(cell_rank.alloc(OD_LEVELS * ((size_t)fc + c)));
+            SCAL_TRY(cell_pts.alloc(OD_LEVELS * ((size_t)fc + c)));
+            return ready.create(EV_DEVICE_ONLY);
+        }
+    };
+    TargetSet set[R];
+    DevBuf<SetCounts> set_cnt;
+    DevBuf<int> ring_tab;
+    int* tab_of(long long k) const { return ring_tab.p + static_cast<int>(k % R) * 4 * RING_TAB; }
+    std::atomic<long long> n_prepared{0}, n_stepped{0};
+    std::atomic<long long> prepared_for[R];
     LMStore lm;
-    DevBuf<int> cell_cnt, cell_start, cell_rank;
-    DevBuf<float4> cell_pts;
-    int* cell_cnt_of(int k, int l) const { return cell_cnt.p + (k * OD_LEVELS + l) * OD_H; }
-    int* cell_start_of(int k, int l) const { return cell_start.p + (k * OD_LEVELS + l) * OD_START_STRIDE; }
-    int* cell_rank_of(int k, int l) const { return cell_rank.p + (size_t)l * (feat_cap + cap) + (k ? feat_cap : 0); }
-    float4* cell_pts_of(int k, int l) const { return cell_pts.p + (size_t)l * (feat_cap + cap) + (k ? feat_cap : 0); }
-    CellIndex cell_index(int k) const {
-        CellIndex ci;
-        for (int l = 0; l < OD_LEVELS; ++l) ci.start[l] = cell_start_of(k, l), ci.pts[l] = cell_pts_of(k, l);
-        return ci;
-    }
-    DevBuf<int> ring_tab;
-    int tab_cur = 0;
     DevBuf<OdomCounters> d_C;
     PinBuf<LMState> h_st;
-    PinBuf<OdomCounters> h_up;
     HostStage hs;
     bool adapter_active = false, adapter_solve = false;
     BlockAdapter blocks;
@@ -480,30 +481,31 @@
     *out = nullptr;
     SCAL_TRY(select_device(cfg->device));
     auto* c = new scal_odom();
+    for (auto& pf : c->prepared_for) pf.store(-1);
     c->cfg = *cfg;
     c->cap = cfg->max_points;
     c->feat_cap = 120 * 64;
     int rc = SCAL_OK;
     auto A = [&](int r) { if (rc == SCAL_OK) rc = r; };
     A(c->lm.alloc(36 * 64));
-    A(c->aos.alloc((size_t)c->cap * 4));
-    A(c->sharp.alloc(c->lm.slot_cap)); A(c->flat.alloc(c->lm.slot_cap));
-    A(c->less_sharp.alloc(c->feat_cap)); A(c->corner_last.alloc(c->feat_cap));
-    A(c->less_flat.alloc(c->cap)); A(c->surf_last.alloc(c->cap));
-    A(c->cell_cnt.alloc(2 * OD_LEVELS * OD_H)); A(c->cell_start.alloc(2 * OD_LEVELS * OD_START_STRIDE));
-    A(c->cell_rank.alloc(OD_LEVELS * ((size_t)c->feat_cap + c->cap))); A(c->cell_pts.alloc(OD_LEVELS * ((size_t)c->feat_cap + c->cap)));
-    A(c->ring_tab.alloc(8 * RING_TAB));
+    A(c->aos.alloc(((size_t)2 * c->lm.slot_cap + c->feat_cap + c->cap) * 4));
+    for (int i = 0; i < scal_odom::R; ++i) A(c->set[i].alloc(c->lm.slot_cap, c->feat_cap, c->cap));
+    A(c->set_cnt.alloc(scal_odom::R));
+    A(c->ring_tab.alloc(scal_odom::R * 4 * RING_TAB));
     A(c->blocks.alloc(c->lm.slot_cap));
-    A(c->d_C.alloc(1)); A(c->h_st.alloc(scal_odom::MAX_STEPS)); A(c->h_up.alloc(1));
+    A(c->d_C.alloc(1)); A(c->h_st.alloc(scal_odom::MAX_STEPS));
     if (rc == SCAL_OK) rc = lm_check_residency<LMNoHook, LMNoHook>(c->cfg.device);
     if (rc == SCAL_OK) rc = c->stream.acquire(c->cfg.device, stage_lane(layout, STAGE_ODOM));
     for (int k = 0; k < scal_odom::MAX_STEPS && rc == SCAL_OK; ++k) rc = c->ev[k].create(hipEventDisableTiming);
     if (rc == SCAL_OK) {
         rc = c->lm.init(c->stream);
         if (rc == SCAL_OK && op_memset_async(c->d_C.p, 0, sizeof(OdomCounters), c->stream) != hipSuccess) rc = SCAL_E_HIP;
-        if (rc == SCAL_OK) rc = c->cell_cnt.zero(c->stream);
-        if (rc == SCAL_OK) rc = c->cell_start.zero(c->stream);
-        SCAL_LAUNCH("k_odom_init_pose", k_odom_init_pose, dim3(1), dim3(256), 0, c->stream, c->lm.d_st.p, c->ring_tab.p);
+        if (rc == SCAL_OK) rc = c->set_cnt.zero(c->stream);
+        for (int i = 0; i < scal_odom::R && rc == SCAL_OK; ++i) {
+            rc = c->set[i].cell_cnt.zero(c->stream);
+            if (rc == SCAL_OK) rc = c->set[i].cell_start.zero(c->stream);
+        }
+        SCAL_LAUNCH("k_odom_init_pose", k_odom_init_pose, dim3(1), dim3(256), 0, c->stream, c->lm.d_st.p, c->ring_tab.p, c->d_C.p);
         if (rc == SCAL_OK && op_stream_synchronize(c->stream) != hipSuccess) rc = SCAL_E_HIP;
     }
     if (rc != SCAL_OK) {
@@ -520,69 +522,111 @@
 extern "C" void scal_odom_destroy(scal_odom_t* c) {
     if (!c) return;
     (void)hipSetDevice(c->cfg.device);
+    for (int i = 0; i < scal_odom::R; ++i)
+        if (c->set[i].prep_stream && c->set[i].prep_stream != c->stream) (void)op_event_synchronize(c->set[i].ready);
     if (c->stream) (void)op_stream_synchronize(c->stream);
     delete c;
 }
 
 namespace {
 
-int launch_handover(scal_odom* c, int slot, hipEvent_t ev);
+int odom_prepare(scal_odom* c, hipStream_t ps, OdomPrepArgs a, long long k = -1) {
+    constexpr int R = scal_odom::R;
+    if (k < 0) k = c->n_prepared.load();
+    const long long stepped = c->n_stepped.load();
+    if (k < stepped || k - stepped > R - 2) {
+        set_error("scal_odom: scan %lld cannot be prepared with %lld steps queued (at most %d scans prepared and not stepped)", k, stepped, R - 1);
+        return SCAL_E_STATE;
+    }
+    scal_odom::TargetSet& T = c->set[k % R];
+    if (ps != c->stream && k >= R - 1) SCAL_HIP(op_stream_wait_event(ps, c->ev[(k - R + 1) % scal_odom::MAX_STEPS], 0));
+    a.o_sharp = T.sharp.v(), a.o_flat = T.flat.v(), a.o_less = T.less_sharp.v(), a.o_less_flat = T.less_flat.v();
+    a.cnt = c->set_cnt.p + (k % R);
+    a.slot_cap = c->lm.slot_cap, a.feat_cap = c->feat_cap;
+    a.nbs = std::max(1, div_up(c->lm.slot_cap, 256)), a.nbf = std::max(1, div_up(c->feat_cap, 256));
+    a.tab = c->tab_of(k);
+    for (int t = 0; t < 2; ++t)
+        for (int l = 0; l < OD_LEVELS; ++l) a.cell_cnt[t][l] = T.cell_cnt_of(t, l), a.cell_rank[t][l] = T.cell_rank_of(t, l);
+    const dim3 grid_lf(a.nbf + std::max(1, div_up(c->cap, 256)));
+    SCAL_LAUNCH("k_odom_prepare", k_odom_prepare, dim3(2 * a.nbs + a.nbf + std::max(1, div_up(a.cap, 256))), dim3(256), 0, ps, a);
+    SCAL_LAUNCH("k_odom_cellscan", k_odom_cellscan, dim3(2 * OD_LEVELS), dim3(1024), 0, ps, T.cell_cnt.p, T.cell_start.p);
+    CellFillArgs f;
+    f.in[0] = T.less_sharp.cv(), f.in[1] = T.less_flat.cv();
+    f.d_n[0] = &a.cnt->n_less_sharp, f.d_n[1] = &a.cnt->n_less_flat;
+    for (int t = 0; t < 2; ++t)
+        for (int l = 0; l < OD_LEVELS; ++l) f.rank[t][l] = T.cell_rank_of(t, l), f.start[t][l] = T.cell_start_of(t, l), f.pts[t][l] = T.cell_pts_of(t, l);
+    f.nb0 = a.nbf;
+    SCAL_LAUNCH("k_odom_cellfill", k_odom_cellfill, grid_lf, dim3(256), 0, ps, f);
+    SCAL_HIP(hipGetLastError());
+    if (ps != c->stream) SCAL_HIP(op_event_record(T.ready, ps));
+    T.prep_stream = ps;
+    c->prepared_for[k % R].store(k);
+    if (c->n_prepared.load() < k + 1) c->n_prepared.store(k + 1);
+    return SCAL_OK;
+}
+
+int odom_prepare_from_features(scal_odom* c, scal_features_t* feat, bool own_stream, long long k = -1) {
+    FeatDeviceView v = features_view(feat);
+    if (v.device != c->cfg.device) {
+        set_error("features context lives on device %d, odometry context on %d", v.device, c->cfg.device);
+        return SCAL_E_ARG;
+    }
+    OdomPrepArgs a{};
+    a.sharp = v.sharp_xyzi, a.flat = v.flat_xyzi, a.less = v.less_xyzi;
+    a.less_flat_aos = nullptr, a.less_flat = CSoA4{v.lfx, v.lfy, v.lfz, v.lfi};
+    a.n_sharp = &v.P->n_sharp, a.n_flat = &v.P->n_flat, a.n_less = &v.P->n_less_sharp, a.n_less_flat = &v.P->n_less_flat;
+    a.cap = std::min(c->cap, v.cap);
+    hipStream_t ps = own_stream ? static_cast<hipStream_t>(c->stream) : v.stream;
+    SCAL_TRY(features_wait_done(feat, ps));
+    SCAL_TRY(odom_prepare(c, ps, a, k));
+    return features_note_reader(feat, ps);
+}
+
+int launch_publish(scal_odom* c, long long j) {
+    hipStream_t s = c->stream;
+    const int slot = static_cast<int>(j % scal_odom::MAX_STEPS);
+    SCAL_LAUNCH("k_odom_publish", k_odom_publish, dim3(1), dim3(256), 0, s, j > 0 ? c->tab_of(j - 1) : static_cast<int*>(nullptr), c->lm.d_st.p,
+                c->h_st.p + slot, c->lm.lm_sync.p);
+    SCAL_HIP(hipGetLastError());
+    SCAL_HIP(op_event_record(c->ev[slot], s));
+    return SCAL_OK;
+}
+
+int wait_prepared(scal_odom* c, long long j) {
+    if (c->prepared_for[j % scal_odom::R].load() != j) {
+        set_error("scal_odom: no prepared scan to step");
+        return SCAL_E_STATE;
+    }
+    scal_odom::TargetSet& Q = c->set[j % scal_odom::R];
+    if (Q.prep_stream != c->stream) SCAL_HIP(op_stream_wait_event(c->stream, Q.ready, 0));
+    return SCAL_OK;
+}
+
 int odom_enqueue(scal_odom* c) {
+    constexpr int R = scal_odom::R;
     hipStream_t s = c->stream;
     OdomCounters* C = c->d_C.p;
     LMState* st = c->lm.d_st.p;
     FactorSoA F = c->lm.factors();
-    const bool solve = c->systemInited;
+    const long long j = c->n_stepped.load();
+    SCAL_TRY(wait_prepared(c, j));
+    const bool solve = c->systemInited && j > 0;
     c->systemInited = true;
-    const int slot = c->next_slot;
-    c->next_slot = (c->next_slot + 1) % scal_odom::MAX_STEPS;
     if (solve) {
+        const scal_odom::TargetSet &Q = c->set[j % R], &T = c->set[(j - 1) % R];
         for (int outer = 0; outer < 2; ++outer) {
             {
-                SCAL_LAUNCH("k_odom_assoc", k_odom_assoc, dim3(std::max(1, c->lm.slot_cap)), dim3(256), 0, s, c->sharp.cv(), c->flat.cv(),
-                                   c->corner_last.cv(), c->surf_last.cv(), st, C, outer, F, c->cell_index(0), c->cell_index(1), c->ring_tab.p + c->tab_cur * 4 * RING_TAB);
+                SCAL_LAUNCH("k_odom_assoc", k_odom_assoc, dim3(std::max(1, c->lm.slot_cap)), dim3(256), 0, s, Q.sharp.cv(), Q.flat.cv(), T.less_sharp.cv(),
+                            T.less_flat.cv(), st, C, c->set_cnt.p + (j % R), c->set_cnt.p + ((j - 1) % R), outer, F, T.cell_index(0), T.cell_index(1), c->tab_of(j - 1));
             }
             {
                                 launch_lm_solve(s, F, &C->n_slots, st, &C->enable, c->lm.partials.p, c->lm.lm_sync.p, outer, nullptr, LMNoHook(), LMNoHook(), "k_lm_solve_odom");
             }
         }
     }
-    SCAL_TRY(launch_handover(c, slot, c->ev[slot]));
-    c->pending.push_back({slot, solve});
-    return SCAL_OK;
-}
-
-int launch_handover(scal_odom* c, int slot, hipEvent_t ev) {
-    hipStream_t s = c->stream;
-    OdomCounters* C = c->d_C.p;
-    LMState* st = c->lm.d_st.p;
-    {
-        HandoverArgs h;
-        h.in[0] = c->less_sharp.cv(), h.in[1] = c->less_flat.cv();
-        h.d_n[0] = &C->n_less_sharp, h.d_n[1] = &C->n_less_flat;
-        h.out[0] = c->corner_last.v(), h.out[1] = c->surf_last.v();
-        h.d_n_out[0] = &C->n_corner_last, h.d_n_out[1] = &C->n_surf_last;
-        h.cap[0] = c->feat_cap, h.cap[1] = c->cap;
-        h.nb0 = std::max(1, div_up(c->feat_cap, 256));
-        h.tab_write = c->ring_tab.p + (c->tab_cur ^ 1) * 4 * RING_TAB;
-        h.tab_reset = c->ring_tab.p + c->tab_cur * 4 * RING_TAB;
-        h.st = st, h.host_st = c->h_st.p + slot, h.sync = c->lm.lm_sync.p;
-        for (int k = 0; k < 2; ++k)
-            for (int l = 0; l < OD_LEVELS; ++l) h.cell_cnt[k][l] = c->cell_cnt_of(k, l), h.cell_rank[k][l] = c->cell_rank_of(k, l);
-        const dim3 grid(h.nb0 + std::max(1, div_up(c->cap, 256)));
-        SCAL_LAUNCH("k_odom_handover", k_odom_handover, grid, dim3(256), 0, s, h);
-        c->tab_cur ^= 1;
-        if (ev) SCAL_HIP(op_event_record(ev, s));
-        SCAL_LAUNCH("k_odom_cellscan", k_odom_cellscan, dim3(2 * OD_LEVELS), dim3(1024), 0, s, c->cell_cnt.p, c->cell_start.p);
-        CellFillArgs f;
-        f.in[0] = c->corner_last.cv(), f.in[1] = c->surf_last.cv();
-        f.d_n[0] = &C->n_corner_last, f.d_n[1] = &C->n_surf_last;
-        for (int k = 0; k < 2; ++k)
-            for (int l = 0; l < OD_LEVELS; ++l) f.rank[k][l] = c->cell_rank_of(k, l), f.start[k][l] = c->cell_start_of(k, l), f.pts[k][l] = c->cell_pts_of(k, l);
-        f.nb0 = h.nb0;
-        SCAL_LAUNCH("k_odom_cellfill", k_odom_cellfill, grid, dim3(256), 0, s, f);
-    }
-    SCAL_HIP(hipGetLastError());
+    SCAL_TRY(launch_publish(c, j));
+    c->pending.push_back({static_cast<int>(j % scal_odom::MAX_STEPS), solve});
+    c->n_stepped.store(j + 1);
     return SCAL_OK;
 }
 
@@ -633,26 +677,18 @@
     SCAL_HIP(op_stream_synchronize(s));
     c->hs.finish();
     (void)c->hs.reserve(((size_t)2 * c->lm.slot_cap + c->feat_cap + c->cap) * 16 + 4096);
-    OdomCounters& H = *c->h_up.p;
-    OdomCounters fresh;
-    std::memset(&fresh, 0, sizeof fresh);
-    fresh.n_sharp = n_sharp, fresh.n_flat = n_flat, fresh.n_less_sharp = n_less_sharp, fresh.n_less_flat = n_less_flat, fresh.enable = 1;
-    H = fresh;
-    const size_t off = offsetof(OdomCounters, n_sharp);
-    SCAL_HIP(op_memcpy_async(reinterpret_cast<char*>(c->d_C.p) + off, reinterpret_cast<char*>(&H) + off, sizeof(OdomCounters) - off,
-                            hipMemcpyHostToDevice, s));
-    auto up = [&](const float* src, int n, SoAStore& dst) -> int {
-        if (n > 0) {
-            SCAL_HIP(c->hs.h2d(c->aos.p, src, sizeof(float) * 4 * n, s));
-            launch_deinterleave(s, c->aos.p, n, dst.v());
-        }
-        return SCAL_OK;
-    };
-    SCAL_TRY(up(sharp, n_sharp, c->sharp));
-    SCAL_TRY(up(flat, n_flat, c->flat));
-    SCAL_TRY(up(less_sharp, n_less_sharp, c->less_sharp));
-    SCAL_TRY(up(less_flat, n_less_flat, c->less_flat));
-    return SCAL_OK;
+    float* d[4] = {c->aos.p, c->aos.p + (size_t)4 * c->lm.slot_cap, c->aos.p + (size_t)8 * c->lm.slot_cap,
+                   c->aos.p + (size_t)4 * (2 * c->lm.slot_cap + c->feat_cap)};
+    const float* h[4] = {sharp, flat, less_sharp, less_flat};
+    const int n[4] = {n_sharp, n_flat, n_less_sharp, n_less_flat};
+    OdomPrepArgs a{};
+    for (int i = 0; i < 4; ++i) {
+        if (n[i] > 0) SCAL_HIP(c->hs.h2d(d[i], h[i], sizeof(float) * 4 * n[i], s));
+        a.n_host[i] = n[i];
+    }
+    a.sharp = d[0], a.flat = d[1], a.less = d[2], a.less_flat_aos = d[3];
+    a.cap = c->cap;
+    return odom_prepare(c, s, a);
 }
 
 extern "C" int scal_odom_step(scal_odom_t* c, const float* sharp, int n_sharp, const float* less_sharp, int n_less_sharp, const float* flat,
@@ -687,23 +723,8 @@
         set_error("scal_odom_enqueue_features: %d steps are queued and not collected", scal_odom::MAX_STEPS);
         return SCAL_E_STATE;
     }
-    FeatDeviceView v = features_view(feat);
-    if (v.device != c->cfg.device) {
-        set_error("features context lives on device %d, odometry context on %d", v.device, c->cfg.device);
-        return SCAL_E_ARG;
-    }
-    SCAL_HIP(hipSetDevice(c->cfg.device));
-    hipStream_t s = c->stream;
-    OdomGatherArgs a;
-    a.sharp = v.sharp_xyzi, a.flat = v.flat_xyzi, a.less = v.less_xyzi;
-    a.less_flat = CSoA4{v.lfx, v.lfy, v.lfz, v.lfi};
-    a.n_sharp = &v.P->n_sharp, a.n_flat = &v.P->n_flat, a.n_less = &v.P->n_less_sharp, a.n_less_flat = &v.P->n_less_flat;
-    a.o_sharp = c->sharp.v(), a.o_flat = c->flat.v(), a.o_less = c->less_sharp.v(), a.o_less_flat = c->less_flat.v();
-    a.slot_cap = c->lm.slot_cap, a.feat_cap = c->feat_cap, a.cap = std::min(c->cap, v.cap);
-    a.nbs = std::max(1, div_up(c->lm.slot_cap, 256)), a.nbf = std::max(1, div_up(c->feat_cap, 256));
-    SCAL_TRY(features_wait_done(feat, s));
-    SCAL_LAUNCH("k_odom_gather", k_odom_gather, dim3(2 * a.nbs + a.nbf + std::max(1, div_up(a.cap, 256))), dim3(256), 0, s, a, c->d_C.p);
-    SCAL_TRY(features_note_reader(feat, s));
+    SCAL_HIP(hipSetDevice(c->cfg.device));
+    SCAL_TRY(odom_prepare_from_features(c, feat, false));
     return odom_enqueue(c);
 }
 
@@ -724,6 +745,27 @@
     }
     SCAL_TRY(scal_odom_enqueue_features(c, feat));
     return odom_collect(c, q_lc, t_lc, q_w, t_w, stats);
+}
+
+int scal::odom_prepare_features(scal_odom_t* c, scal_features_t* feat, bool own_stream, long long scan) {
+    if (!c || !feat) {
+        set_error("odom_prepare_features: null argument");
+        return SCAL_E_ARG;
+    }
+    SCAL_HIP(hipSetDevice(c->cfg.device));
+    return odom_prepare_from_features(c, feat, own_stream, scan);
+}
+int scal::odom_enqueue_prepared(scal_odom_t* c) {
+    if (!c) {
+        set_error("odom_enqueue_prepared: null argument");
+        return SCAL_E_ARG;
+    }
+    if (static_cast<int>(c->pending.size()) >= scal_odom::MAX_STEPS) {
+        set_error("odom_enqueue_prepared: %d steps are queued and not collected", scal_odom::MAX_STEPS);
+        return SCAL_E_STATE;
+    }
+    SCAL_HIP(hipSetDevice(c->cfg.device));
+    return odom_enqueue(c);
 }
 
 extern "C" int scal_odom_adapter_begin(scal_odom_t* c, const float* sharp, int n_sharp, const float* less_sharp, int n_less_sharp, const float* flat,
@@ -749,7 +791,7 @@
     SCAL_HIP(op_stream_synchronize(s));
     for (int i = 0; i < 4; ++i) q_last_curr[i] = c->h_st.p->x[i];
     for (int i = 0; i < 3; ++i) t_last_curr[i] = c->h_st.p->x[4 + i];
-    c->adapter_solve = c->systemInited;
+    c->adapter_solve = c->systemInited && c->n_stepped.load() > 0;
     c->systemInited = true;
     *need_solve = c->adapter_solve ? 1 : 0;
     c->adapter_active = true;
@@ -772,8 +814,12 @@
     LMState* st = c->lm.d_st.p;
     FactorSoA F = c->lm.factors();
     SCAL_TRY(c->blocks.set_pose(c->stream, c->lm.d_st.p->x, q_last_curr, t_last_curr));
-    SCAL_LAUNCH("k_odom_assoc", k_odom_assoc, dim3(std::max(1, c->lm.slot_cap)), dim3(256), 0, s, c->sharp.cv(), c->flat.cv(), c->corner_last.cv(),
-                     c->surf_last.cv(), st, C, std::min(c->outer_next, 1), F, c->cell_index(0), c->cell_index(1), c->ring_tab.p + c->tab_cur * 4 * RING_TAB);
+    const long long j = c->n_stepped.load();
+    SCAL_TRY(wait_prepared(c, j));
+    const scal_odom::TargetSet &Q = c->set[j % scal_odom::R], &T = c->set[(j - 1) % scal_odom::R];
+    SCAL_LAUNCH("k_odom_assoc", k_odom_assoc, dim3(std::max(1, c->lm.slot_cap)), dim3(256), 0, s, Q.sharp.cv(), Q.flat.cv(), T.less_sharp.cv(), T.less_flat.cv(),
+                st, C, c->set_cnt.p + (j % scal_odom::R), c->set_cnt.p + ((j - 1) % scal_odom::R), std::min(c->outer_next, 1), F, T.cell_index(0), T.cell_index(1),
+                c->tab_of(j - 1));
     c->outer_next++;
     SCAL_TRY(c->blocks.compact(s, F, &C->n_slots));
     SCAL_HIP(op_stream_synchronize(s));
@@ -819,10 +865,10 @@
     SCAL_HIP(hipSetDevice(c->cfg.device));
     c->adapter_active = false;
     SCAL_TRY(c->blocks.set_pose(c->stream, c->lm.d_st.p->x, q_last_curr, t_last_curr));
-    const int slot = c->next_slot;
-    c->next_slot = (c->next_slot + 1) % scal_odom::MAX_STEPS;
-    SCAL_TRY(launch_handover(c, slot, c->ev[slot]));
-    c->pending.push_back({slot, c->adapter_solve});
+    const long long j = c->n_stepped.load();
+    SCAL_TRY(launch_publish(c, j));
+    c->pending.push_back({static_cast<int>(j % scal_odom::MAX_STEPS), c->adapter_solve});
+    c->n_stepped.store(j + 1);
     double q_lc[4], t_lc[3];
     return odom_collect(c, q_lc, t_lc, q_w_curr, t_w_curr, nullptr);
 }
diff --git a/sc-a-loam_amd/csrc/pipeline.cpp b/sc-a-loam_amd/csrc/pipeline.cpp
--- a/sc-a-loam_amd/csrc/pipeline.cpp
+++ b/sc-a-loam_amd/csrc/pipeline.cpp
@@ -26,6 +26,7 @@
 }
 const int B_AHEAD = env_int("SCALOAM_PIPE_B_AHEAD", 2, 1, 3);
 const int PF_AHEAD = env_int("SCALOAM_PIPE_PF_AHEAD", 3, 1, 3);
+const bool PAIR = env_int("SCALOAM_PIPE_PAIR", 1, 0, 1) != 0;
 
 const bool TIMING = env_int("SCALOAM_PIPE_TIMING", 0, 0, 1) != 0;
 struct HostTimer {
@@ -73,6 +74,7 @@
     std::mutex mu;
     std::condition_variable cv;
     long long pushed = 0, a_run = 0, a_done = 0, pf_done = 0, b_enq = 0, b_coll = 0, c_enq = 0, c_coll = 0, d_ins = 0, d_coll = 0, popped = 0;
+    long long pairs = 0;
     int pop_waiting = 0;
     bool drain_req = false, drained = true;
     bool stop = false;
@@ -143,38 +145,63 @@
 
 void front_thread(scal_pipeline* p) {
     std::unique_lock<std::mutex> lk(p->mu);
+    auto ready = [&](long long k) {
+        if (p->pushed <= k) return false;
+        const long long old = k - p->ring;
+        if (old >= 0 && (p->c_coll <= old || p->b_enq <= old || (p->sc_on() && p->d_ins <= old))) return false;
+        return p->b_enq + ODOM_TARGET_SETS - 1 > k;
+    };
+    auto runnable = [&](long long k) { return ready(k) && k - p->c_enq < PF_AHEAD; };
+    auto pairable = [&](long long k) { return PAIR && p->S == 1 && !p->r(k).host && ready(k + 1) && !p->r(k + 1).host; };
     for (;;) {
         const long long k = p->a_done;
-        p->cv.wait(lk, [&] {
-            if (p->stop || p->err) return true;
-            if (p->pushed <= k) return false;
-            const long long old = k - p->ring;
-            if (old >= 0 && (p->c_coll <= old || p->b_enq <= old || (p->sc_on() && p->d_ins <= old))) return false;
-            return k - p->c_enq < PF_AHEAD;
-        });
+        p->cv.wait(lk, [&] { return p->stop || p->err || runnable(k); });
         if (p->stop || p->err) return;
-        const Rec& rc = p->r(k);
-        const int slot = static_cast<int>(k % p->ring);
+        const int np = (pairable(k) && runnable(k + 1)) ? 2 : 1;
+        const Rec* rc[2] = {&p->r(k), &p->r(k + 1)};
+        const int slot[2] = {static_cast<int>(k % p->ring), static_cast<int>((k + 1) % p->ring)};
         lk.unlock();
-        int st = p->tm_front.run(0, "A: features_run", [&] {
-            return p->for_all([&](int q) {
-                scal_features_t* reg = p->regs[q][slot];
-                return rc.host ? scal_features_enqueue_host(reg, rc.h_xyz[q], rc.n[q], rc.stride) : scal_features_run_device(reg, rc.d_xyz[q], rc.n[q], rc.stride);
-            });
+        auto stage_a = [&](int i, int q) {
+            scal_features_t* reg = p->regs[q][slot[i]];
+            SCAL_TRY(rc[i]->host ? scal_features_enqueue_host(reg, rc[i]->h_xyz[q], rc[i]->n[q], rc[i]->stride)
+                                 : scal_features_run_device(reg, rc[i]->d_xyz[q], rc[i]->n[q], rc[i]->stride));
+            return rc[i]->host ? SCAL_OK : odom_prepare_features(p->od[q], reg, false, k + i);
+        };
+        int st = p->tm_front.run(0, "A: features_run + B: prepare", [&]() -> int {
+            if (np == 1) return p->for_all([&](int q) { return stage_a(0, q); });
+            Recorder recs[2];
+            Recorder* ptr[2] = {&recs[0], &recs[1]};
+            int r2 = SCAL_OK;
+            for (int i = 0; i < 2 && r2 == SCAL_OK; ++i) {
+                g_recorder = ptr[i];
+                r2 = stage_a(i, 0);
+                g_recorder = nullptr;
+            }
+            if (r2 != SCAL_OK) {
+                for (int i = 0; i < 2; ++i) (void)recs[i].flush();
+                return r2;
+            }
+            if (zip_and_launch(ptr, 2) != hipSuccess) {
+                set_error("scal_pipeline: a batched launch failed: %s", hipGetErrorString(hipGetLastError()));
+                return SCAL_E_HIP;
+            }
+            return SCAL_OK;
         });
         if (st == SCAL_OK) {
             lk.lock();
-            p->a_run = k + 1;
+            p->a_run = k + np;
+            if (np == 2) p->pairs++;
             p->cv.notify_all();
             lk.unlock();
-            st = p->tm_front.run(1, "C: prefetch, lane 0 half", [&] { return p->for_all([&](int q) { return scal_map_prefetch_begin(p->mp[q], p->regs[q][slot]); }); });
+            for (int i = 0; i < np && st == SCAL_OK; ++i)
+                st = p->tm_front.run(1, "C: prefetch, lane 0 half", [&] { return p->for_all([&](int q) { return scal_map_prefetch_begin(p->mp[q], p->regs[q][slot[i]]); }); });
         }
         lk.lock();
         if (st != SCAL_OK) {
             p->fail(st);
             return;
         }
-        p->a_done = k + 1;
+        p->a_done = k + np;
         p->cv.notify_all();
     }
 }
@@ -258,9 +285,15 @@
         int st = SCAL_OK;
         if (what == B_ENQ) {
             const long long k = p->b_enq;
+            const bool host = p->r(k).host;
             const int slot = static_cast<int>(k % p->ring);
             lk.unlock();
-            st = p->tm_odom.run(0, "B: odom_enqueue_features", [&] { return p->for_all([&](int q) { return scal_odom_enqueue_features(p->od[q], p->regs[q][slot]); }); });
+            st = p->tm_odom.run(0, "B: odom_enqueue_prepared", [&] {
+                return p->for_all([&](int q) {
+                    if (host) SCAL_TRY(odom_prepare_features(p->od[q], p->regs[q][slot], true, k));
+                    return odom_enqueue_prepared(p->od[q]);
+                });
+            });
             lk.lock();
             if (st == SCAL_OK) p->b_enq = k + 1;
         } else {
@@ -908,6 +941,13 @@
     return static_cast<int>(p->pushed - p->popped);
 }
 
+extern "C" int scal_debug_pipeline_pairs(scal_pipeline_t* p, long long* pairs) {
+    if (!p || !pairs) return SCAL_E_ARG;
+    std::lock_guard<std::mutex> lk(p->mu);
+    *pairs = p->pairs;
+    return SCAL_OK;
+}
+
 static bool seq_ok(scal_pipeline_t* p, int q) { return p && q >= 0 && q < p->S; }
 extern "C" scal_sc_t* scal_pipeline_sc(scal_pipeline_t* p) { return p ? p->sc[0] : nullptr; }
 extern "C" scal_map_t* scal_pipeline_map(scal_pipeline_t* p) { return p ? p->mp[0] : nullptr; }
```

New measurement: 4277. -1.9%, worse.
